# Traneptora/hydrium

Measured on AMD Instinct MI355X. Metric: Mpixel/s encode (8K RGB, default q), higher is better.
Workload: dtype f32

## Files before the change

### hydrium_amd/csrc/hip/device_api.hip

```cpp
#include <hip/hip_runtime.h>

#include <stdint.h>
#include <stdio.h>
#include <stdlib.h>
#include <string.h>

#include <atomic>
#include <condition_variable>
#include <functional>
#include <mutex>
#include <thread>
#include <vector>

#include "../../../include/hydrium_amd.h"
#include "hydk_common.h"
#include "../hyd_sample_fmt.h"

#pragma clang fp contract(off)

namespace hydk {
hipError_t launch_transform(const HydkLfJob *d_jobs, int num_slots, unsigned fmt_mask, int xmode, uint32_t *status,
                            uint2 *part_info, int plog, hipStream_t stream);
hipError_t launch_tables(const uint32_t *hist, HydkTables *tabs, const uint32_t *alpha_max, int nclusters, int first_slot,
                         int num_slots, uint32_t alpha_floor, const uint32_t *alpha_floor_dev, const uint32_t *lf_hist,
                         HydkLfStream *lf_streams, void *lf_work, const HydkLfJob *jobs_all, hipStream_t stream);
hipError_t launch_export(const HydkLfJob *d_jobs, const HydkTables *tabs, const uint32_t *group_bits, const HydkLfStream *lf_streams,
                         const uint8_t *payload, const uint64_t *hf_total, const uint8_t *lf_packed,
                         const unsigned long long *lf_total, const uint32_t *status, int num_slots, int lf_coded, uint8_t *dst,
                         uint64_t capacity, int view, hipStream_t stream);
hipError_t launch_rans(const HydkLfJob *d_jobs, const uint32_t *sym_count, const HydkTables *tabs, uint32_t *bitbuf,
                       uint32_t bit_pitch_words, uint32_t *group_bits, int num_slots, const uint32_t *status,
                       hipStream_t stream);
hipError_t launch_rans_deferred(const HydkLfJob *d_jobs, const uint32_t *sym_count, const HydkTables *tabs, uint16_t *aux,
                                uint16_t *flags, uint32_t aux_pitch, uint32_t *final_state, uint32_t *group_bits,
                                int num_slots, const uint32_t *status, hipStream_t stream);
hipError_t launch_rans_lanes(const HydkLfJob *d_jobs, const uint32_t *sym_count, const HydkTables *tabs, uint16_t *aux,
                             uint16_t *flags, uint32_t aux_pitch, uint32_t *final_state, uint32_t *group_bits,
                             int nclusters, int num_slots, const uint32_t *status, const uint32_t *lf_hist,
                             HydkLfStream *lf_streams, void *lf_work, hipStream_t stream);
hipError_t launch_lf_front(const HydkLfJob *d_jobs, unsigned long long *recs, uint32_t *hist, void *work, int num_slots,
                           hipStream_t stream);
hipError_t launch_lf_back(const HydkLfJob *d_jobs, const unsigned long long *recs, HydkLfStream *streams, uint32_t *bits,
                          void *work, int num_slots, hipStream_t stream);
hipError_t launch_rans_emit(const HydkLfJob *d_jobs, const uint32_t *sym_count, const uint16_t *aux, const uint16_t *flags,
                            uint32_t aux_pitch, const uint32_t *final_state, const uint32_t *group_bits, uint64_t *offsets,
                            uint8_t *payload, int num_slots, uint32_t *status, uint64_t *total, uint64_t payload_cap,
                            hipStream_t stream);
hipError_t launch_frame_begin(const HydkLfJob *host_jobs, HydkLfJob *d_jobs, int count, uint32_t *accum, size_t accum_words,
                              hipStream_t stream);
hipError_t launch_publish(const uint64_t *total, uint64_t *h_total, const unsigned long long *lf_total,
                          unsigned long long *h_lf_total, const uint32_t *status, uint32_t *h_status, hipStream_t stream);
hipError_t transform_footprint(int fmt, int storage, int xmode, int *lds_bytes, int *registers);
hipError_t launch_scan(const uint32_t *group_bits, int count, uint64_t *offsets, uint64_t *total, uint8_t *payload,
                       uint64_t payload_cap, int clear_shared_words, uint32_t *status, hipStream_t stream);
hipError_t launch_pack(const uint32_t *bitbuf, uint32_t bit_pitch_words, const uint32_t *group_bits, const uint64_t *offsets,
                       uint8_t *payload, int count, const uint32_t *status, hipStream_t stream);
size_t lf_work_bytes();
hipError_t launch_batch_extents(const void *blob, int frames, void *extents, hipStream_t stream);
hipError_t launch_lf_coder(const HydkLfJob *d_jobs, unsigned long long *recs, uint32_t *hist, HydkLfStream *streams,
                           uint32_t *bits, void *work, int num_slots, hipStream_t stream);
hipError_t launch_lf_gather(HydkLfStream *streams, const uint32_t *bits, uint32_t *packed, unsigned long long *total,
                            int num_slots, hipStream_t stream);
hipError_t launch_lf_huffman_only(const uint32_t *hist, HydkLfStream *stream_out, uint32_t *codes, hipStream_t stream);
hipError_t launch_lut_selftest(const uint16_t *in_lut16, const float *bias_lut, int linear_light, int xmode,
                               uint32_t *mismatches, hipStream_t stream);
}

#define ST_OK 0
#define ST_NOMEM (-13)
#define ST_API_ERROR (-14)
#define ST_INTERNAL_ERROR (-15)

static_assert(sizeof(HydAmdBlobHeader) == 64 && sizeof(HydAmdBlobSlot) == 16 + 36 + 12 + 256 + 4608 + sizeof(HydkLfStream) &&
                  sizeof(HydAmdBlobSlot) % 16 == 0,
              "blob records are laid out by k_export_frame word by word");
static_assert(HYDAMD_MAX_CLUSTERS == HYDK_MAX_CLUSTERS && HYDAMD_ALPHABET == HYDK_ALPHABET &&
                  HYDAMD_GROUPS_PER_LFG == HYDK_GROUPS_PER_LFG && HYDAMD_LF_CODES == HYDK_LF_CODES,
              "public and kernel-side table shapes must agree");

namespace {

constexpr int kStaging = 2;
constexpr int kSplitSlots = 2;
int split_slots() {
    static const int n = [] {
        const char *e = getenv("HYDAMD_K1_SPLIT_SLOTS");
        const int v = e ? atoi(e) : kSplitSlots;
        return v < 0 ? 0 : v > 256 ? 256 : v;
    }();
    return n;
}
constexpr size_t kDbgPlane = (size_t)2048 * 2048;

char g_global_error[256] = "";

struct TimedLaunch {
    int cls;
    hipEvent_t start, stop;
};

}

struct HydAmdContext {
    int device = 0;
    int max_slots = 0;
    int linear_light = 0;
    int use_luts = 2;
    int best_register_mode = 2;
    int curve_gathers = 0;
    uint64_t published_pixels = 0;
    uint64_t seen_bytes = 0, seen_pixels = 0;
    int register_luts_ok = 0;
    int rans_lanes = 0;
    uint32_t tok_cap = HYDK_DEFAULT_TOKEN_CAP;
    bool caps_forced = false;
    unsigned grown_ahead = 0;
    uint32_t rec_bytes = 4;
    uint32_t bit_pitch_words = 0;
    int want_transform = 0, want_entropy = 0;
    bool slot_lanes[HYDAMD_MAX_LF_GROUPS] = {};
    bool slot_lane_chain[HYDAMD_MAX_LF_GROUPS] = {};
    unsigned overflow_reruns = 0;
    uint32_t alpha_floor = 0;
    const uint32_t *alpha_floor_dev = nullptr;
    unsigned num_presets = 1;
    int scheme = 0;
    int nclusters = 9;
    hipStream_t own_stream = nullptr;
    hipStream_t stream = nullptr;
    char error[256] = "";

    char *tokens = nullptr;
    uint32_t *bitbuf = nullptr;
    uint16_t *rans_aux = nullptr;
    uint16_t *rans_flags = nullptr;
    uint32_t *rans_final = nullptr;
    uint32_t *rbits_total = nullptr;
    HydkTables *tables = nullptr;
    int32_t *dc = nullptr;
    uint32_t *hist = nullptr;
    uint32_t *sym_count = nullptr;
    uint2 *part_info = nullptr;
    uint32_t *group_bits = nullptr;
    uint64_t *offsets = nullptr;
    uint64_t *total = nullptr;
    uint32_t *status = nullptr;
    uint32_t *alpha_max = nullptr;
    uint32_t *bad_slots = nullptr;
    bool bad_per_slot = false;
    HydkLfJob *d_jobs = nullptr;
    HydkLfJob *h_jobs = nullptr;
    HydkLfJob *h_jobs_ring[4] = {nullptr, nullptr, nullptr, nullptr};
    hipEvent_t jobs_uploaded[4] = {nullptr, nullptr, nullptr, nullptr};
    unsigned frame_counter = 0;
    int jobs_idx = 0;
    uint16_t *in_lut8 = nullptr, *in_lut16 = nullptr;
    float *bias_lut = nullptr;
    uint8_t *payload = nullptr;
    size_t payload_cap = 0;

    int lf_on_device = 1;
    unsigned long long *lf_recs = nullptr;
    uint32_t *lf_hist = nullptr;
    uint32_t *lf_codes = nullptr;
    char *lf_work = nullptr;
    HydkLfStream *lf_streams = nullptr;
    uint32_t *lf_bits = nullptr;
    uint32_t *lf_packed = nullptr;
    unsigned long long *lf_total = nullptr;
    unsigned long long *h_lf_total_pinned = nullptr;
    uint64_t h_lf_total = 0;
    hipStream_t lf_stream = nullptr;
    hipEvent_t lf_fork = nullptr, lf_join = nullptr;
    bool lf_pending = false;
    bool lf_need_gather = false;
    bool lf_results_valid = false;
    hipEvent_t lf_ready = nullptr;
    int lf_slots = 0;
    int transformed = 0, coded = 0, lf_coded = 0;
    int host_staged = 0;
    float *dbg_xyb = nullptr, *dbg_dct = nullptr;
    int32_t *dbg_quant = nullptr;

    void *pinned[kStaging] = {nullptr, nullptr};
    char *d_arena = nullptr;
    size_t arena_tile = 0;
    size_t staging_cap = 0;
    hipEvent_t staged[kStaging] = {nullptr, nullptr};
    int staging_next = 0;
    hipStream_t copy_stream = nullptr;
    bool copy_stream_shared = false;
    hipEvent_t frame_fence = nullptr;
    bool copy_needs_fence = false;

    uint64_t h_total = 0;
    uint32_t h_status = 0;
    int slots_finished = 0;
    int slots_per_frame = 0;
    uint8_t slot_frame_first[HYDAMD_MAX_LF_GROUPS] = {};
    uint8_t slot_frame_groups[HYDAMD_MAX_LF_GROUPS] = {};
    bool results_valid = false;
    uint32_t *accum = nullptr;
    size_t accum_words = 0;
    bool accum_stale = true;
    bool lf_total_unpublished = false;
    bool status_published = false;
    uint64_t *h_total_pinned = nullptr;
    uint32_t *h_status_pinned = nullptr;

    hipEvent_t peer_event = nullptr;
    uint32_t *peer_floor = nullptr;
    unsigned long long *verify_sums = nullptr;

    void *own_blob = nullptr;
    size_t own_blob_cap = 0;
    void *stage_blob = nullptr;
    size_t stage_blob_cap = 0;
    uint8_t *stage_host = nullptr;
    size_t stage_host_cap = 0;
    int stage_slots = 0;
    HydAmdAssembler *assembler = nullptr;
    void *batch_extents = nullptr;
    size_t batch_extents_cap = 0;

    bool profiling = false;
    std::vector<TimedLaunch> timed;
    double prof_ms[HYDAMD_K_COUNT] = {0, 0, 0, 0, 0};
    uint64_t prof_n[HYDAMD_K_COUNT] = {0, 0, 0, 0, 0};
};

namespace {

int fail(HydAmdContext *ctx, int code, const char *what, hipError_t e = hipSuccess) {
    char *dst = ctx ? ctx->error : g_global_error;
    if (e != hipSuccess)
        snprintf(dst, 256, "%s: %s", what, hipGetErrorString(e));
    else
        snprintf(dst, 256, "%s", what);
    return code;
}

#define HIP_TRY(ctx, call)                                                          \
    do {                                                                            \
        hipError_t e__ = (call);                                                    \
        if (e__ != hipSuccess)                                                      \
            return fail(ctx, e__ == hipErrorOutOfMemory ? ST_NOMEM : ST_INTERNAL_ERROR, #call, e__); \
    } while (0)

float host_linearize(float x) {
    if (x <= 0.0404482362771082f)
        return 0.07739938080495357f * x;
    return 0.003094300919832f + x * (-0.009982599f + x * (0.72007737769f + 0.2852804880f * x));
}

float host_bias(float v) {
    const float x = v + 0.0037930732552754493f;
    union {
        float f;
// ... 776 lines not shown

int hydamd_set_xyb_mode(HydAmdContext *ctx, int mode) {
    if (!ctx)
        return ST_API_ERROR;
    if (recorded_but_not_transformed(ctx))
        return fail(ctx, ST_API_ERROR, "the XYB mode cannot change between recording an LF group and its transform stage");
    if (mode < ctx->best_register_mode || mode > 2)
        return fail(ctx, ST_API_ERROR, "XYB mode not available (it must have passed the bit-exactness self-test)");
    ctx->use_luts = mode;
    return ST_OK;
}

int hydamd_forget_content(HydAmdContext *ctx) {
    if (!ctx)
        return ST_API_ERROR;
    ctx->seen_bytes = ctx->seen_pixels = 0;
    return ST_OK;
}

int hydamd_set_curve_gathers(HydAmdContext *ctx, int mode) {
    if (!ctx)
        return ST_API_ERROR;
    if (mode < 0 || mode > 2)
        return fail(ctx, ST_API_ERROR, "curve gathers: 0 by content, 1 always, 2 never");
    ctx->curve_gathers = mode;
    return ST_OK;
}

int hydamd_set_rans_waves(HydAmdContext *ctx, int waves) {
    if (!ctx)
        return ST_API_ERROR;
    if (waves >= 1 && waves <= 3) {
        ctx->rans_lanes = retired_rans_form(waves);
        return ST_OK;
    }
    if (waves < 4 || waves > 6)
        return fail(ctx, ST_API_ERROR, "entropy-stage form must be 4 (wave per group) or 5 (lane per group; 6 is accepted as a synonym)");
    ctx->rans_lanes = waves - 4;
    return ST_OK;
}

int hydamd_begin_frame(HydAmdContext *ctx, unsigned num_presets) {
    if (!ctx)
        return ST_API_ERROR;
    if (num_presets < 1 || num_presets > HYDAMD_MAX_LF_GROUPS || num_presets == 128)
        return fail(ctx, ST_API_ERROR, "unsupported number of LF groups per frame (1..255 except 128)");
    HIP_TRY(ctx, hipSetDevice(ctx->device));
    ctx->num_presets = num_presets;
    if (num_presets * 9 <= 256) {
        ctx->scheme = 0;
        ctx->nclusters = 9;
    } else if (num_presets * 3 <= 256) {
        ctx->scheme = 1;
        ctx->nclusters = 3;
    } else if (num_presets * 2 <= 256) {
        ctx->scheme = 2;
        ctx->nclusters = 2;
    } else {
        ctx->scheme = 3;
        ctx->nclusters = 1;
    }
    {
        const uint32_t seen = g_outgrown.load(std::memory_order_relaxed);
        const bool tok = (seen & HYDK_STATUS_TOKENS) && ctx->tok_cap < HYDK_TOKENS_PER_GROUP;
        const bool pay = (seen & HYDK_STATUS_PAYLOAD) && ctx->payload_cap < payload_bound(ctx);
        if ((tok || pay) && !ctx->caps_forced && hipStreamQuery(ctx->stream) == hipSuccess &&
            (!ctx->lf_stream || hipStreamQuery(ctx->lf_stream) == hipSuccess)) {
            if (tok)
                ctx->tok_cap = HYDK_TOKENS_PER_GROUP;
            const int st = alloc_frame_arrays(ctx, pay ? payload_bound(ctx) : ctx->payload_cap);
            if (st != ST_OK)
                return st;
            ctx->grown_ahead++;
        }
        (void)hipGetLastError();
    }
    ctx->results_valid = false;
    ctx->slots_finished = 0;
    ctx->slots_per_frame = 0;
    ctx->transformed = ctx->coded = ctx->lf_coded = 0;
    ctx->want_transform = ctx->want_entropy = 0;
    ctx->host_staged = 0;
    ctx->lf_need_gather = false;
    ctx->lf_results_valid = false;
    ctx->lf_slots = 0;
    HIP_TRY(ctx, hipEventRecord(ctx->frame_fence, ctx->stream));
    ctx->copy_needs_fence = true;
    ctx->jobs_idx = (int)(ctx->frame_counter++ & 3u);
    HIP_TRY(ctx, hipEventSynchronize(ctx->jobs_uploaded[ctx->jobs_idx]));
    ctx->h_jobs = ctx->h_jobs_ring[ctx->jobs_idx];
    memset(ctx->h_jobs, 0, (size_t)ctx->max_slots * sizeof(HydkLfJob));
    ctx->accum_stale = true;
    ctx->alpha_floor = 0;
    ctx->alpha_floor_dev = nullptr;
    return ST_OK;
}

int hydamd_encode_lf_group(HydAmdContext *ctx, int slot, const void *const src[3], ptrdiff_t row_stride,
                           ptrdiff_t pixel_stride, int sample_fmt, size_t width, size_t height, unsigned preset) {
    int st = check_slot(ctx, slot);
    if (st != ST_OK)
        return st;
    if (!src || !src[0] || !src[1] || !src[2])
        return fail(ctx, ST_API_ERROR, "null pixel pointer");
    return record_lf_group(ctx, slot, src, row_stride, pixel_stride, sample_fmt, width, height, preset);
}

int hydamd_encode_lf_group_host(HydAmdContext *ctx, int slot, const void *const src[3], ptrdiff_t row_stride,
                                ptrdiff_t pixel_stride, int sample_fmt, size_t width, size_t height, unsigned preset) {
    int st = check_slot(ctx, slot);
    if (st != ST_OK)
        return st;
    if (!src || !src[0] || !src[1] || !src[2])
        return fail(ctx, ST_API_ERROR, "null pixel pointer");
    if (width == 0 || height == 0 || width > 2048 || height > 2048)
        return fail(ctx, ST_API_ERROR, "LF group must be between 1 and 2048 pixels in each direction");
    if (!hyd_fmt_is_host(sample_fmt))
        return fail(ctx, ST_API_ERROR, "Invalid Sample Format");
    HIP_TRY(ctx, hipSetDevice(ctx->device));
    const size_t ss = hyd_fmt_bytes(sample_fmt);
    const size_t bytes = width * height * 3 * ss;
    st = ensure_staging(ctx, (size_t)2048 * 2048 * 3 * ss);
    if (st != ST_OK)
        return st;
    const int k = ctx->staging_next;
    ctx->staging_next = (k + 1) % kStaging;
    HIP_TRY(ctx, hipEventSynchronize(ctx->staged[k]));
    if (sample_fmt == HYDK_FMT_U8)
        gather_packed((uint8_t *)ctx->pinned[k], src, row_stride, pixel_stride, width, height);
    else if (sample_fmt == HYDK_FMT_U16)
        gather_packed((uint16_t *)ctx->pinned[k], src, row_stride, pixel_stride, width, height);
    else
        gather_packed((float *)ctx->pinned[k], src, row_stride, pixel_stride, width, height);
    char *base = ctx->d_arena + (size_t)slot * ctx->arena_tile;
    if (ctx->copy_needs_fence) {
        HIP_TRY(ctx, hipStreamWaitEvent(ctx->copy_stream, ctx->frame_fence, 0));
        ctx->copy_needs_fence = false;
    }
    HIP_TRY(ctx, hipMemcpyAsync(base, ctx->pinned[k], bytes, hipMemcpyHostToDevice, ctx->copy_stream));
    HIP_TRY(ctx, hipEventRecord(ctx->staged[k], ctx->copy_stream));
    HIP_TRY(ctx, hipStreamWaitEvent(ctx->stream, ctx->staged[k], 0));
    const void *dsrc[3] = {base, base + ss, base + 2 * ss};
    st = record_lf_group(ctx, slot, dsrc, (ptrdiff_t)(3 * width), 3, sample_fmt, width, height, preset);
    if (st == ST_OK && slot + 1 > ctx->host_staged)
        ctx->host_staged = slot + 1;
    return st;
}

int hydamd_encode_image(HydAmdContext *ctx, const void *const src[3], ptrdiff_t row_stride, ptrdiff_t pixel_stride,
                        int sample_fmt, size_t width, size_t height) {
    if (!ctx)
        return ST_API_ERROR;
    if (!src || !src[0] || !src[1] || !src[2])
        return fail(ctx, ST_API_ERROR, "null pixel pointer");
    if (width == 0 || height == 0)
        return fail(ctx, ST_API_ERROR, "empty image");
    const size_t lfx = (width + 2047) >> 11, lfy = (height + 2047) >> 11;
    if (lfx * lfy > (size_t)ctx->max_slots)
        return fail(ctx, ST_API_ERROR, "context has too few LF-group slots for this image");
    if (!hyd_fmt_is_device(sample_fmt))
        return fail(ctx, ST_API_ERROR, "Invalid Sample Format");
    if (!hyd_fmt_layout_ok(sample_fmt, src, pixel_stride))
        return fail(ctx, ST_API_ERROR, HYD_FMT_NV12_LAYOUT_MSG);
    int st = hydamd_begin_frame(ctx, (unsigned)(lfx * lfy));
    for (size_t ty = 0; ty < lfy && st == ST_OK; ty++)
        for (size_t tx = 0; tx < lfx && st == ST_OK; tx++) {
// ... 43 lines not shown
            ctx->slot_frame_first[first + i] = (uint8_t)first;
            ctx->slot_frame_groups[first + i] = (uint8_t)lf_groups[k];
        }
    ctx->slots_per_frame = -1;
    return ST_OK;
}

int hydamd_encode_image_batch(HydAmdContext *ctx, int frames, const void *const *src , ptrdiff_t row_stride,
                              ptrdiff_t pixel_stride, int sample_fmt, size_t width, size_t height) {
    if (!ctx)
        return ST_API_ERROR;
    if (!src || frames < 1)
        return fail(ctx, ST_API_ERROR, "null pixel pointer");
    if (width == 0 || height == 0)
        return fail(ctx, ST_API_ERROR, "empty image");
    if (!hyd_fmt_is_device(sample_fmt))
        return fail(ctx, ST_API_ERROR, "Invalid Sample Format");
    for (int f = 0; f < frames; f++)
        if (src[3 * (size_t)f + 1] && !hyd_fmt_layout_ok(sample_fmt, src + 3 * (size_t)f, pixel_stride))
            return fail(ctx, ST_API_ERROR, HYD_FMT_NV12_LAYOUT_MSG);
    const size_t lfx = (width + 2047) >> 11, lfy = (height + 2047) >> 11, n = lfx * lfy;
    int st = hydamd_begin_batch(ctx, (unsigned)n, frames);
    for (int f = 0; f < frames && st == ST_OK; f++) {
        const void *const *s3 = src + 3 * (size_t)f;
        if (!s3[0] || !s3[1] || !s3[2])
            return fail(ctx, ST_API_ERROR, "null pixel pointer");
        for (size_t ty = 0; ty < lfy && st == ST_OK; ty++)
            for (size_t tx = 0; tx < lfx && st == ST_OK; tx++) {
                const void *p[3];
                hyd_fmt_origin(sample_fmt, s3, row_stride, pixel_stride, tx * 2048, ty * 2048, p);
                const size_t w = width - tx * 2048 < 2048 ? width - tx * 2048 : 2048;
                const size_t h = height - ty * 2048 < 2048 ? height - ty * 2048 : 2048;
                st = hydamd_encode_lf_group(ctx, (int)((size_t)f * n + ty * lfx + tx), p, row_stride, pixel_stride, sample_fmt, w, h,
                                            (unsigned)(ty * lfx + tx));
            }
    }
    if (st == ST_OK)
        st = hydamd_finish_frame(ctx, (int)((size_t)frames * n));
    return st;
}

static int transform_range(HydAmdContext *ctx, int first, int count) {
    unsigned mask = 0;
    for (int i = first; i < first + count; i++) {
        if (ctx->h_jobs[i].width == 0)
            return fail(ctx, ST_API_ERROR, "an LF-group slot of this frame was never submitted");
        mask |= 1u << (ctx->h_jobs[i].storage ? HYDK_FMT_F32 + (int)ctx->h_jobs[i].storage : ctx->h_jobs[i].fmt);
    }
    ctx->status_published = false;
    HIP_TRY(ctx, hydk::launch_frame_begin(ctx->h_jobs + first, ctx->d_jobs + first, count,
                                          ctx->accum_stale ? ctx->accum : nullptr, ctx->accum_words, ctx->stream));
    ctx->accum_stale = false;
    HIP_TRY(ctx, hipEventRecord(ctx->jobs_uploaded[ctx->jobs_idx], ctx->stream));
    ScopedTimer timer(ctx, HYDAMD_K_TRANSFORM);
    int xmode = ctx->use_luts;
    if (xmode < 2) {
        bool dense = ctx->curve_gathers == 2;
        if (ctx->curve_gathers == 0 && ctx->seen_pixels)
            dense = (double)ctx->seen_bytes > 0.75 * (double)ctx->seen_pixels;
        if (dense)
            xmode += 3;
    }
    static const bool split_on = !(getenv("HYDAMD_K1_SPLIT") && atoi(getenv("HYDAMD_K1_SPLIT")) == 0);
    static const int split_log = getenv("HYDAMD_K1_SPLIT_LOG") && atoi(getenv("HYDAMD_K1_SPLIT_LOG")) == 1 ? 1 : 2;
    const int plog = split_on && count <= split_slots() && ctx->tok_cap % 64 == 0 ? split_log : 0;
    HIP_TRY(ctx, hydk::launch_transform(ctx->d_jobs + first, count, mask, xmode, ctx->status, ctx->part_info, plog, ctx->stream));
    return ST_OK;
}

#ifdef HYD_TEST_HOOKS
static int lf_drop() {
    static const int v = getenv("HYDAMD_DEBUG_LF_DROP") ? atoi(getenv("HYDAMD_DEBUG_LF_DROP")) : 0;
    return v;
}
#else
static constexpr int lf_drop() { return 0; }
#endif
static int ensure_lf_stream(HydAmdContext *ctx) {
    if (!ctx->lf_stream)
        HIP_TRY(ctx, hipStreamCreateWithFlags(&ctx->lf_stream, hipStreamNonBlocking));
    return ST_OK;
}

static int lf_range(HydAmdContext *ctx, int first, int count, bool forked) {
    if (forked) {
        const int st = ensure_lf_stream(ctx);
        if (st != ST_OK)
            return st;
    }
    hipStream_t where = forked ? ctx->lf_stream : ctx->stream;
    ctx->status_published = false;
    if (forked) {
        HIP_TRY(ctx, hipEventRecord(ctx->lf_fork, ctx->stream));
        HIP_TRY(ctx, hipStreamWaitEvent(ctx->lf_stream, ctx->lf_fork, 0));
    }
    ScopedTimer timer(ctx, HYDAMD_K_LF, where);
    HIP_TRY(ctx, hydk::launch_lf_coder(ctx->d_jobs + first, ctx->lf_recs + (size_t)first * HYDK_LF_SYMBOLS,
                                       ctx->lf_hist + (size_t)first * HYDK_LF_CODES, ctx->lf_streams + first,
                                       ctx->lf_bits + (size_t)first * HYDK_LF_BITWORDS,
                                       ctx->lf_work + (size_t)first * hydk::lf_work_bytes(), count, where));
    ctx->lf_pending = ctx->lf_pending || forked;
    ctx->lf_need_gather = true;
    return ST_OK;
}

int hydamd_run_transform(HydAmdContext *ctx, int num_slots) {
    if (!ctx)
        return ST_API_ERROR;
    if (num_slots < 1 || num_slots > ctx->max_slots)
        return fail(ctx, ST_API_ERROR, "slot count out of range");
    HIP_TRY(ctx, hipSetDevice(ctx->device));
    ctx->results_valid = false;
    if (num_slots > ctx->want_transform)
        ctx->want_transform = num_slots;
    if (num_slots > ctx->transformed) {
        const int st = transform_range(ctx, ctx->transformed, num_slots - ctx->transformed);
        if (st != ST_OK)
            return st;
        ctx->transformed = num_slots;
    }
    if (ctx->lf_on_device == 1 && num_slots > ctx->lf_coded) {
        const int st = lf_range(ctx, ctx->lf_coded, num_slots - ctx->lf_coded, true);
        if (st != ST_OK)
            return st;
        ctx->lf_coded = num_slots;
    }
    return ST_OK;
}

static int join_lf(HydAmdContext *ctx, int num_slots, bool totals_follow = false) {
    if (num_slots > 0 && ctx->lf_on_device == 2 && num_slots > ctx->lf_coded) {
        const int st = lf_range(ctx, ctx->lf_coded, num_slots - ctx->lf_coded, false);
        if (st != ST_OK)
            return st;
        ctx->lf_coded = num_slots;
    }
    if (num_slots > 0 && ctx->lf_need_gather) {
        hipStream_t where = ctx->lf_pending ? ctx->lf_stream : ctx->stream;
        if (!(lf_drop() & 8))
        HIP_TRY(ctx, hydk::launch_lf_gather(ctx->lf_streams, ctx->lf_bits, ctx->lf_packed, ctx->lf_total, num_slots, where));
        if (totals_follow && !ctx->lf_pending)
            ctx->lf_total_unpublished = true;
        else
            HIP_TRY(ctx, hydk::launch_publish(nullptr, nullptr, ctx->lf_total, ctx->h_lf_total_pinned, nullptr, nullptr, where));
        HIP_TRY(ctx, hipEventRecord(ctx->lf_ready, where));
        ctx->lf_slots = num_slots;
        ctx->lf_need_gather = false;
    }
    if (ctx->lf_pending) {
        HIP_TRY(ctx, hipEventRecord(ctx->lf_join, ctx->lf_stream));
        HIP_TRY(ctx, hipStreamWaitEvent(ctx->stream, ctx->lf_join, 0));
        ctx->lf_pending = false;
    }
    return ST_OK;
}

static int replay_frame(HydAmdContext *ctx) {
    const int recorded = ctx->want_transform > ctx->transformed ? ctx->want_transform : ctx->transformed;
    for (int i = 0; i < ctx->max_slots; i++)
        if (ctx->h_jobs[i].width)
            bind_slot_buffers(ctx, i);
    ctx->accum_stale = true;
    const int entropy = ctx->want_entropy;
    ctx->transformed = ctx->coded = ctx->lf_coded = 0;
    ctx->results_valid = false;
    if (recorded > 0) {
        const int st = hydamd_run_transform(ctx, recorded);
        if (st != ST_OK)
            return st;
    }
    if (entropy > 0)
        return hydamd_run_entropy(ctx, entropy);
    return ST_OK;
}

static int resolve_overflow(HydAmdContext *ctx, uint32_t status, bool *again) {
    *again = false;
    if (!(status & HYDK_STATUS_OVERFLOW))
        return ST_OK;
    if (status & HYDK_STATUS_LAYOUT)
        return fail(ctx, ST_INTERNAL_ERROR, "float LF group in a context laid out for integer token records");
    if (ctx->lf_stream)
        HIP_TRY(ctx, hipStreamSynchronize(ctx->lf_stream));
    size_t payload_cap = ctx->payload_cap;
    if (status & HYDK_STATUS_TOKENS) {
// ... 565 lines not shown
                         : "vcc");
            acc = fl;
        } else {
            x = x * 1664525u + 1013904223u + row;
        }
        if (LDS) {
            const uint32_t sadr = lds0 + (__umulhi(x, lds_bytes > 2u ? lds_bytes - 2u : 1u) & ~1u);
            asm volatile("ds_read_u16 %0, %1\n\ts_waitcnt lgkmcnt(0)" : "=v"(slot) : "v"(sadr) : "memory");
            x ^= slot;
        }
        if (!VALU)
            __builtin_amdgcn_s_sleep(1);
#pragma unroll
        for (int i = 0; i < 96; i++)
            asm volatile("" : "+v"(hold[i]));
    }
    uint32_t r = x ^ acc;
#pragma unroll
    for (int i = 0; i < 96; i++)
        r ^= hold[i];
    if (r == 0xFFFFFFFFu && sink)
        *sink = r;
}
}
static int debug_skip() {
    static const int v = getenv("HYDAMD_DEBUG_SKIP") ? atoi(getenv("HYDAMD_DEBUG_SKIP")) : 0;
    return v;
}
static int env_int(const char *name, int dflt) {
    const char *v = getenv(name);
    return v && *v ? atoi(v) : dflt;
}
static void launch_chain_standins(HydAmdContext *ctx, int count) {
    static const int wgs = env_int("HYDAMD_DEBUG_SLEEP_WGS", 1);
    static const int lds = env_int("HYDAMD_DEBUG_SLEEP_LDS", 0);
    static const unsigned long long ticks = 100ull * (unsigned long long)env_int("HYDAMD_DEBUG_SLEEP_US", 2500);
    static const int regs = env_int("HYDAMD_DEBUG_SLEEP_VGPRS", 0);
    static const int steps = env_int("HYDAMD_DEBUG_STANDIN_STEPS", 30000);
    static const char *kind = getenv("HYDAMD_DEBUG_STANDIN") ? getenv("HYDAMD_DEBUG_STANDIN") : "sleep";
    const dim3 grid(wgs > 0 ? wgs * count : 1);
#define HYDK_STANDIN(MODE, THREADS)                                                                                         \
    do {                                                                                                                    \
        if (lds > 65536)                                                                                                    \
            (void)hipFuncSetAttribute((const void *)k_chain_standin, hipFuncAttributeMaxDynamicSharedMemorySize, lds);      \
        hipLaunchKernelGGL(k_chain_standin, grid, dim3(THREADS), (size_t)lds, ctx->stream, MODE, (uint32_t)steps,           \
                           (uint32_t)lds, (uint32_t *)nullptr);                                                             \
    } while (0)
    if (!strcmp(kind, "valu"))
        HYDK_STANDIN(1, 64);
    else if (!strcmp(kind, "lds"))
        HYDK_STANDIN(2, 64);
    else if (!strcmp(kind, "both"))
        HYDK_STANDIN(3, 64);
    else if (!strcmp(kind, "valu4"))
        HYDK_STANDIN(5, 256);
    else if (regs >= 160) {
        if (lds > 65536)
            (void)hipFuncSetAttribute((const void *)k_sleep_probe_regs160, hipFuncAttributeMaxDynamicSharedMemorySize, lds);
        hipLaunchKernelGGL(k_sleep_probe_regs160, grid, dim3(64), (size_t)lds, ctx->stream, ticks, (uint32_t *)nullptr);
    } else if (regs >= 124) {
        if (lds > 65536)
            (void)hipFuncSetAttribute((const void *)k_sleep_probe_regs124, hipFuncAttributeMaxDynamicSharedMemorySize, lds);
        hipLaunchKernelGGL(k_sleep_probe_regs124, grid, dim3(64), (size_t)lds, ctx->stream, ticks, (uint32_t *)nullptr);
    } else if (regs >= 100) {
        if (lds > 65536)
            (void)hipFuncSetAttribute((const void *)k_sleep_probe_regs104, hipFuncAttributeMaxDynamicSharedMemorySize, lds);
        hipLaunchKernelGGL(k_sleep_probe_regs104, grid, dim3(64), (size_t)lds, ctx->stream, ticks, (uint32_t *)nullptr);
    } else if (regs >= 40) {
        if (lds > 65536)
            (void)hipFuncSetAttribute((const void *)k_sleep_probe_regs40, hipFuncAttributeMaxDynamicSharedMemorySize, lds);
        hipLaunchKernelGGL(k_sleep_probe_regs40, grid, dim3(64), (size_t)lds, ctx->stream, ticks, (uint32_t *)nullptr);
    } else {
        if (lds > 65536)
            (void)hipFuncSetAttribute((const void *)k_sleep_probe, hipFuncAttributeMaxDynamicSharedMemorySize, lds);
        hipLaunchKernelGGL(k_sleep_probe, grid, dim3(64), (size_t)lds, ctx->stream, ticks);
    }
#undef HYDK_STANDIN
}
#else
static constexpr int debug_skip() { return 0; }
static void launch_chain_standins(HydAmdContext *, int) {}
#endif

static int entropy_range(HydAmdContext *ctx, int first, int count, bool with_lf_codes) {
    const size_t G = HYDK_GROUPS_PER_LFG, g0 = (size_t)first * G;
    {
        ScopedTimer timer(ctx, HYDAMD_K_TABLES);
        if (!(debug_skip() & 1)) {
        static const bool ride_with_tables = getenv("HYDAMD_LF_CODES_RIDE") && !strcmp(getenv("HYDAMD_LF_CODES_RIDE"), "tables");
        const bool here = with_lf_codes && ride_with_tables;
        HIP_TRY(ctx, hydk::launch_tables(ctx->hist, ctx->tables, ctx->alpha_max, ctx->nclusters, first, count,
                                         ctx->alpha_floor, ctx->alpha_floor_dev,
                                         here ? ctx->lf_hist + (size_t)first * HYDK_LF_CODES : nullptr, ctx->lf_streams + first,
                                         ctx->lf_work + (size_t)first * hydk::lf_work_bytes(), ctx->d_jobs, ctx->stream));
        if (here)
            with_lf_codes = false;
        }
    }
    {
        ScopedTimer timer(ctx, HYDAMD_K_RANS);
        const HydkLfJob *jobs = ctx->d_jobs + first;
        bool any_float = false;
        for (int i = first; i < first + count; i++)
            any_float = any_float || ctx->h_jobs[i].fmt == HYDK_FMT_F32;
        const bool lanes = ctx->rans_lanes && !any_float;
        bool emits = lanes;
        if (with_lf_codes && !lanes)
            return fail(ctx, ST_INTERNAL_ERROR, "LF code construction can only ride with the lane-form entropy stage");
        (void)lanes;
        if (debug_skip() & 16) {
            launch_chain_standins(ctx, count);
        } else if (debug_skip() & 2) {
        } else if (lanes) {
            HIP_TRY(ctx, hydk::launch_rans_lanes(jobs, ctx->sym_count + g0, ctx->tables + first,
                                                 ctx->rans_aux + g0 * ctx->tok_cap, ctx->rans_flags + g0 * (ctx->tok_cap / 16),
                                                 ctx->tok_cap, ctx->rans_final + g0, ctx->group_bits + g0,
                                                 ctx->nclusters, count, ctx->status,
                                                 with_lf_codes ? ctx->lf_hist + (size_t)first * HYDK_LF_CODES : nullptr,
                                                 ctx->lf_streams + first, ctx->lf_work + (size_t)first * hydk::lf_work_bytes(),
                                                 ctx->stream));
        } else if (!any_float && wave_form_defers()) {
            HIP_TRY(ctx, hydk::launch_rans_deferred(jobs, ctx->sym_count + g0, ctx->tables + first, ctx->rans_aux + g0 * ctx->tok_cap,
                                                    ctx->rans_flags + g0 * (ctx->tok_cap / 16), ctx->tok_cap, ctx->rans_final + g0,
                                                    ctx->group_bits + g0, count, ctx->status, ctx->stream));
            emits = true;
        } else {
            const int st = ensure_bitbuf(ctx);
            if (st != ST_OK)
                return st;
            HIP_TRY(ctx, hydk::launch_rans(jobs, ctx->sym_count + g0, ctx->tables + first,
                                           ctx->bitbuf + g0 * ctx->bit_pitch_words, ctx->bit_pitch_words,
                                           ctx->group_bits + g0, count, ctx->status, ctx->stream));
        }
        for (int i = first; i < first + count; i++) {
            ctx->slot_lanes[i] = emits;
            ctx->slot_lane_chain[i] = lanes;
        }
    }
    return ST_OK;
}

int hydamd_run_entropy(HydAmdContext *ctx, int num_slots) {
    if (!ctx)
        return ST_API_ERROR;
    if (num_slots < 1 || num_slots > ctx->max_slots)
        return fail(ctx, ST_API_ERROR, "slot count out of range");
    if (num_slots > ctx->transformed)
        return fail(ctx, ST_API_ERROR, "the entropy stage needs the transform stage of the same slots first");
    HIP_TRY(ctx, hipSetDevice(ctx->device));
    const int count = num_slots * HYDK_GROUPS_PER_LFG;
    ctx->results_valid = false;
    ctx->want_entropy = num_slots;
    int lf_first = -1, lf_count = 0;
    if (num_slots > ctx->coded && ctx->lf_on_device == 2 && ctx->rans_lanes && ctx->lf_coded == ctx->coded && !ctx->lf_pending &&
        !(debug_skip() & 8)) {
        bool any_float = false;
        for (int i = ctx->coded; i < num_slots; i++)
            any_float = any_float || ctx->h_jobs[i].fmt == HYDK_FMT_F32;
        if (!any_float) {
            lf_first = ctx->coded;
            lf_count = num_slots - ctx->coded;
            ScopedTimer timer(ctx, HYDAMD_K_LF);
            if (!(lf_drop() & 1))
            HIP_TRY(ctx, hydk::launch_lf_front(ctx->d_jobs + lf_first, ctx->lf_recs + (size_t)lf_first * HYDK_LF_SYMBOLS,
                                               ctx->lf_hist + (size_t)lf_first * HYDK_LF_CODES,
                                               ctx->lf_work + (size_t)lf_first * hydk::lf_work_bytes(), lf_count, ctx->stream));
        }
    }
    if (num_slots > ctx->coded) {
        const int st = entropy_range(ctx, ctx->coded, num_slots - ctx->coded, lf_count > 0 && !(lf_drop() & 2));
        if (st != ST_OK)
            return st;
        ctx->coded = num_slots;
    }
    if (!(debug_skip() & 4)) {
        ScopedTimer timer(ctx, HYDAMD_K_PACK);
        bool all_emit = true;
        for (int i = 0; i < num_slots; i++)
            all_emit = all_emit && ctx->slot_lane_chain[i];
        if (all_emit)
            HIP_TRY(ctx, hydk::launch_rans_emit(ctx->d_jobs, ctx->sym_count, ctx->rans_aux, ctx->rans_flags, ctx->tok_cap,
                                                ctx->rans_final, ctx->group_bits, ctx->offsets, ctx->payload, num_slots,
                                                ctx->status, ctx->total, ctx->payload_cap, ctx->stream));
        else
            HIP_TRY(ctx, hydk::launch_scan(ctx->group_bits, count, ctx->offsets, ctx->total, ctx->payload, ctx->payload_cap, 1,
                                           ctx->status, ctx->stream));
        for (int first = all_emit ? num_slots : 0; first < num_slots;) {
            int last = first;
            while (last + 1 < num_slots && ctx->slot_lanes[last + 1] == ctx->slot_lanes[first])
                last++;
            const int n = last - first + 1;
            const size_t g0 = (size_t)first * HYDK_GROUPS_PER_LFG;
            if (ctx->slot_lanes[first])
                HIP_TRY(ctx, hydk::launch_rans_emit(ctx->d_jobs + first, ctx->sym_count + g0, ctx->rans_aux + g0 * ctx->tok_cap,
                                                    ctx->rans_flags + g0 * (ctx->tok_cap / 16), ctx->tok_cap,
                                                    ctx->rans_final + g0, ctx->group_bits + g0, ctx->offsets + g0, ctx->payload,
                                                    n, ctx->status, nullptr, 0, ctx->stream));
            else
                HIP_TRY(ctx, hydk::launch_pack(ctx->bitbuf + g0 * ctx->bit_pitch_words, ctx->bit_pitch_words,
                                               ctx->group_bits + g0, ctx->offsets + g0, ctx->payload,
                                               n * HYDK_GROUPS_PER_LFG, ctx->status, ctx->stream));
            first = last + 1;
        }
    }
    if (lf_count > 0) {
        ScopedTimer timer(ctx, HYDAMD_K_LF);
        if (!(lf_drop() & 4))
        HIP_TRY(ctx, hydk::launch_lf_back(ctx->d_jobs + lf_first, ctx->lf_recs + (size_t)lf_first * HYDK_LF_SYMBOLS,
                                          ctx->lf_streams + lf_first, ctx->lf_bits + (size_t)lf_first * HYDK_LF_BITWORDS,
                                          ctx->lf_work + (size_t)lf_first * hydk::lf_work_bytes(), lf_count, ctx->stream));
        ctx->lf_coded = num_slots;
        ctx->lf_need_gather = true;
    }
    {
        const int st = join_lf(ctx, num_slots, true);
        if (st != ST_OK)
            return st;
    }
    {
        uint64_t px = 0;
        for (int i = 0; i < num_slots; i++)
            px += (uint64_t)ctx->h_jobs[i].width * (uint64_t)ctx->h_jobs[i].height;
        ctx->published_pixels = px;
    }
    HIP_TRY(ctx, hydk::launch_publish(ctx->total, ctx->h_total_pinned, ctx->lf_total_unpublished ? ctx->lf_total : nullptr,
                                      ctx->h_lf_total_pinned, ctx->status, ctx->h_status_pinned, ctx->stream));
#ifdef HYD_TEST_HOOKS
    {
        static const int extra = env_int("HYDAMD_DEBUG_EXTRA_LAUNCHES", 0);
        for (int i = 0; i < extra; i++)
            HIP_TRY(ctx, hydk::launch_publish(nullptr, nullptr, nullptr, nullptr, nullptr, nullptr, ctx->stream));
    }
#endif
    if (ctx->lf_total_unpublished)
        HIP_TRY(ctx, hipEventRecord(ctx->lf_ready, ctx->stream));
    ctx->lf_total_unpublished = false;
    ctx->status_published = true;
    ctx->slots_finished = num_slots;
    return ST_OK;
}

int hydamd_submit_lf_group(HydAmdContext *ctx, int slot) {
    int st = check_slot(ctx, slot);
    if (st != ST_OK)
        return st;
    if (slot != ctx->transformed)
        return fail(ctx, ST_API_ERROR, "LF groups are submitted early in slot order, one at a time");
    HIP_TRY(ctx, hipSetDevice(ctx->device));
    ctx->results_valid = false;
    st = transform_range(ctx, slot, 1);
    if (st == ST_OK)
        ctx->transformed = slot + 1;
    return st;
}

int hydamd_run_lf_coder(HydAmdContext *ctx, int num_slots, int last) {
    if (!ctx)
        return ST_API_ERROR;
    if (!ctx->lf_on_device)
        return fail(ctx, ST_API_ERROR, "the LF coder is off");
    if (num_slots < 1 || num_slots > ctx->max_slots)
        return fail(ctx, ST_API_ERROR, "slot count out of range");
    HIP_TRY(ctx, hipSetDevice(ctx->device));
    ctx->results_valid = false;
    if (num_slots > ctx->transformed) {
        const int st = transform_range(ctx, ctx->transformed, num_slots - ctx->transformed);
        if (st != ST_OK)
            return st;
        ctx->transformed = num_slots;
    }
    if (ctx->lf_pending) {
        HIP_TRY(ctx, hipEventRecord(ctx->lf_join, ctx->lf_stream));
        HIP_TRY(ctx, hipStreamWaitEvent(ctx->stream, ctx->lf_join, 0));
        ctx->lf_pending = false;
    }
    if (num_slots > ctx->lf_coded) {
        const int st = lf_range(ctx, ctx->lf_coded, num_slots - ctx->lf_coded, false);
        if (st != ST_OK)
            return st;
        ctx->lf_coded = num_slots;
    }
    return last ? join_lf(ctx, num_slots) : ST_OK;
}

int hydamd_sync_lf(HydAmdContext *ctx) {
    if (!ctx)
        return ST_API_ERROR;
    if (!ctx->lf_on_device || ctx->lf_need_gather || ctx->lf_slots == 0)
        return fail(ctx, ST_API_ERROR, "no finished LF coder run to wait for");
    HIP_TRY(ctx, hipSetDevice(ctx->device));
    HIP_TRY(ctx, hipEventSynchronize(ctx->lf_ready));
    ctx->h_lf_total = *ctx->h_lf_total_pinned;
    ctx->lf_results_valid = true;
    return ST_OK;
}
// ... 176 lines not shown
        for (int c = 0; c < 3; c++)
            rgb[3 * i + c] = (uint8_t)out[c];
    }
    return ST_OK;
}

namespace {
__global__ __launch_bounds__(256) void k_yuv_to_rgb_probe(int matrix, const uint8_t *yuv, uint8_t *rgb, size_t n) {
    const size_t i = (size_t)blockIdx.x * 256u + threadIdx.x;
    if (i >= n)
        return;
    uint32_t out[3];
    hydk_yuv_to_rgb(hydk_yuv_matrix(matrix), yuv[3 * i], yuv[3 * i + 1], yuv[3 * i + 2], out);
    for (int c = 0; c < 3; c++)
        rgb[3 * i + c] = (uint8_t)out[c];
}
}

__attribute__((visibility("default"))) int hydt_yuv_to_rgb_device(int device, int matrix, const uint8_t *yuv, uint8_t *rgb, size_t n) {
    if (matrix < 0 || matrix >= HYDK_YUV_MATRICES || !yuv || !rgb || n == 0 || n >= ((size_t)1 << 31) ||
        hipSetDevice(device) != hipSuccess)
        return ST_API_ERROR;
    uint8_t *d_in = nullptr, *d_out = nullptr;
    hipError_t e = hipMalloc((void **)&d_in, 3 * n);
    if (e == hipSuccess)
        e = hipMalloc((void **)&d_out, 3 * n);
    if (e == hipSuccess)
        e = hipMemcpy(d_in, yuv, 3 * n, hipMemcpyHostToDevice);
    if (e == hipSuccess) {
        hipLaunchKernelGGL(k_yuv_to_rgb_probe, dim3((unsigned)((n + 255) / 256)), dim3(256), 0, nullptr, matrix, d_in, d_out, n);
        e = hipGetLastError();
    }
    if (e == hipSuccess)
        e = hipMemcpy(rgb, d_out, 3 * n, hipMemcpyDeviceToHost);
    (void)hipFree(d_in);
    (void)hipFree(d_out);
    return e == hipSuccess ? ST_OK : ST_API_ERROR;
}
#endif

int hydamd_set_lf_coder(HydAmdContext *ctx, int on_device) {
    if (!ctx)
        return ST_API_ERROR;
    ctx->lf_on_device = on_device == 2 ? 2 : on_device != 0;
    return ST_OK;
}

int hydamd_lf_coder(HydAmdContext *ctx) { return ctx ? ctx->lf_on_device : 0; }

int hydamd_read_lf_stream(HydAmdContext *ctx, int slot, uint8_t lengths[HYDAMD_LF_CODES], uint32_t *alphabet,
                          uint32_t *run_pairs, uint32_t *bit_count) {
    int st = check_slot(ctx, slot);
    if (st != ST_OK)
        return st;
    if (!ctx->lf_on_device || !ctx->lf_results_valid)
        return fail(ctx, ST_API_ERROR, "no device-coded LF stream: the LF coder is off or the frame was not synchronised");
    HydkLfStream h;
    HIP_TRY(ctx, hipMemcpy(&h, ctx->lf_streams + slot, sizeof(h), hipMemcpyDeviceToHost));
    if (h.error)
        return fail(ctx, ST_INTERNAL_ERROR, "LF code construction failed on the device");
    memcpy(lengths, h.lengths, HYDK_LF_CODES);
    if (alphabet)
        *alphabet = h.alphabet;
    if (run_pairs)
        *run_pairs = h.run_pairs;
    if (bit_count)
        *bit_count = h.bit_count;
    return ST_OK;
}

int hydamd_read_lf_bits(HydAmdContext *ctx, int slot, uint8_t *dst, size_t capacity) {
    int st = check_slot(ctx, slot);
    if (st != ST_OK)
        return st;
    if (!ctx->lf_on_device || !ctx->lf_results_valid)
        return fail(ctx, ST_API_ERROR, "no device-coded LF stream: the LF coder is off or the frame was not synchronised");
    if (capacity > (size_t)HYDK_LF_BITWORDS * sizeof(uint32_t))
        return fail(ctx, ST_API_ERROR, "LF bit request too large");
    if (!capacity)
        return ST_OK;
    HydkLfStream h;
    HIP_TRY(ctx, hipMemcpy(&h, ctx->lf_streams + slot, sizeof(h), hipMemcpyDeviceToHost));
    const size_t have = ((size_t)h.bit_count + 7u) / 8u, n = capacity < have ? capacity : have;
    if (n)
        HIP_TRY(ctx, hipMemcpy(dst, ctx->lf_bits + (size_t)slot * HYDK_LF_BITWORDS, n, hipMemcpyDeviceToHost));
    memset(dst + n, 0, capacity - n);
    return ST_OK;
}

size_t hydamd_lf_payload_size(HydAmdContext *ctx) {
    return ctx && ctx->lf_results_valid && ctx->lf_on_device ? (size_t)ctx->h_lf_total : 0;
}

const uint8_t *hydamd_lf_payload_device(HydAmdContext *ctx) { return ctx ? (const uint8_t *)ctx->lf_packed : nullptr; }

int hydamd_read_lf_payload(HydAmdContext *ctx, uint8_t *dst, size_t capacity) {
    if (!ctx || !ctx->lf_on_device || !ctx->lf_results_valid)
        return fail(ctx, ST_API_ERROR, "no device-coded LF stream: the LF coder is off or the frame was not synchronised");
    if (capacity < ctx->h_lf_total)
        return fail(ctx, ST_API_ERROR, "LF payload buffer too small");
    if (ctx->h_lf_total)
        HIP_TRY(ctx, hipMemcpy(dst, ctx->lf_packed, ctx->h_lf_total, hipMemcpyDeviceToHost));
    return ST_OK;
}

int hydamd_read_lf_streams(HydAmdContext *ctx, int first_slot, int count, HydAmdLfInfo *dst) {
    if (!ctx || !ctx->lf_on_device || !ctx->lf_results_valid)
        return fail(ctx, ST_API_ERROR, "no device-coded LF stream: the LF coder is off or the frame was not synchronised");
    if (first_slot < 0 || count < 1 || first_slot + count > ctx->lf_slots)
        return fail(ctx, ST_API_ERROR, "LF-group slot range out of bounds");
    static_assert(sizeof(HydAmdLfInfo) == sizeof(HydkLfStream), "public and kernel-side LF stream records must agree");
    HIP_TRY(ctx, hipMemcpy(dst, ctx->lf_streams + first_slot, (size_t)count * sizeof(HydkLfStream), hipMemcpyDeviceToHost));
    for (int i = 0; i < count; i++)
        if (dst[i].error)
            return fail(ctx, ST_INTERNAL_ERROR, "LF code construction failed on the device");
    return ST_OK;
}

int hydamd_debug_transform_footprint(HydAmdContext *ctx, int sample_fmt, int *lds_bytes, int *registers) {
    if (!ctx || !lds_bytes || !registers || !hyd_fmt_is_device(sample_fmt))
        return ST_API_ERROR;
    HIP_TRY(ctx, hipSetDevice(ctx->device));
    HIP_TRY(ctx, hydk::transform_footprint(fmt_class(sample_fmt), (int)fmt_storage(sample_fmt), ctx->use_luts, lds_bytes, registers));
    return ST_OK;
}

namespace {
__global__ __launch_bounds__(64) void k_clock_probe(unsigned long long *out) {
    const unsigned long long r0 = __builtin_amdgcn_s_memrealtime();
    const unsigned long long c0 = __builtin_amdgcn_s_memtime();
    unsigned long long r1 = r0;
    while (r1 - r0 < 2000ull)
        r1 = __builtin_amdgcn_s_memrealtime();
    const unsigned long long c1 = __builtin_amdgcn_s_memtime();
    if (threadIdx.x == 0) {
        out[0] = c1 - c0;
        out[1] = r1 - r0;
    }
}
}

int hydamd_debug_shader_clock_mhz(HydAmdContext *ctx, double *mhz) {
    if (!ctx || !mhz)
        return ST_API_ERROR;
    HIP_TRY(ctx, hipSetDevice(ctx->device));
    static std::mutex lock;
    static hipStream_t sides[HYDAMD_MAX_PEERS * 2];
    static unsigned long long *pinned[HYDAMD_MAX_PEERS * 2];
    if (ctx->device < 0 || ctx->device >= HYDAMD_MAX_PEERS * 2)
        return fail(ctx, ST_API_ERROR, "device index out of range");
    std::lock_guard<std::mutex> hold(lock);
    hipStream_t &side = sides[ctx->device];
    unsigned long long *&h = pinned[ctx->device];
    if (!side)
        HIP_TRY(ctx, hipStreamCreateWithFlags(&side, hipStreamNonBlocking));
    if (!h)
        HIP_TRY(ctx, hipHostMalloc((void **)&h, 2 * sizeof(unsigned long long), hipHostMallocDefault));
    hipLaunchKernelGGL(k_clock_probe, dim3(1), dim3(64), 0, side, h);
    HIP_TRY(ctx, hipGetLastError());
    HIP_TRY(ctx, hipStreamSynchronize(side));
    *mhz = h[1] ? 100.0 * (double)h[0] / (double)h[1] : 0.0;
    return ST_OK;
}

int hydamd_debug_lf_code(HydAmdContext *ctx, const uint32_t hist[HYDAMD_LF_CODES], uint8_t lengths[HYDAMD_LF_CODES],
                         uint32_t codes[HYDAMD_LF_CODES], uint32_t *alphabet, uint32_t *error) {
    if (!ctx)
        return ST_API_ERROR;
// ... 92 lines not shown
```

### hydrium_amd/csrc/hip/kernels.hip

```cpp
#include <hip/hip_runtime.h>
#include <stdint.h>

#include "hydk_common.h"
#include "hydk_edges.h"
#include <atomic>
#include <type_traits>

#pragma clang fp contract(off)

namespace {

constexpr int kThreads = 256;
#ifndef HYDK_K1_WAVES
#define HYDK_K1_WAVES 4
#endif
#ifndef HYDK_K1_GATHER
#define HYDK_K1_GATHER 0x10
#endif
#ifndef HYDK_K1_WAVELOCAL
#define HYDK_K1_WAVELOCAL 1
#endif
#ifndef HYDK_K1_SKIP
#define HYDK_K1_SKIP 0
#endif
// ... 1017 lines not shown
                    uint32_t token, rbits, residue;
                    if (FMT != HYDK_FMT_F32) {
                        const uint32_t fb = __float_as_uint((float)value) >> 22;
                        const bool big = value >= 16u;
                        token = big ? fb - 246u : value;
                        rbits = big ? (fb >> 1) - 128u : 0u;
                        residue = __builtin_amdgcn_ubfe(value, 0u, rbits);
                    } else if (value < 16) {
                        token = value;
                        rbits = 0;
                        residue = 0;
                    } else {
                        const int nb = 30 - __clz((int)value);
                        rbits = (uint32_t)nb;
                        residue = value & ((1u << nb) - 1u);
                        token = 16u + (((uint32_t)(nb - 3) << 1) | ((value >> nb) & 1u));
                    }
#if HYDK_K1_TRIM
                    const uint32_t bin = umad24(cluster, (uint32_t)kHistW, FMT == HYDK_FMT_F32 ? min(token, (uint32_t)kHistW - 1u) : token);
#else
                    const uint32_t bin = cluster * kHistW + (FMT == HYDK_FMT_F32 ? min(token, (uint32_t)kHistW - 1u) : token);
#endif
                    store_record<FMT>(tok, goff + p, token, cluster, bin, rbits, residue);
                    rb_sum += rbits;
                    atomicAdd(&s_hist[bin], 1u);
                    const uint32_t here = coef != 0 ? 1u : 0u;
                    remaining -= here;
                    prev = is_count ? (uint32_t)(nz_total <= 4u) : here;
                    if (++j == n) {
                        seg_at++;
                        visit = visit == 2u ? 0u : visit + 1u;
                        seg = s_seg[seg_at];
                        n = seg.z & 0xffu;
                        nz_total = remaining = seg.z >> 8;
                        j = 0;
                    }
                }
            }
        }
        goff += strip_total;
        __syncthreads();
    }

    __syncthreads();
    uint32_t top_token = 0;
    for (int i = t; i < HYDK_MAX_CLUSTERS * kHistW; i += kThreads) {
        const uint32_t v = s_hist[i];
        if (v) {
            atomicAdd(&job.hist[(i / kHistW) * HYDK_ALPHABET + i % kHistW], v);
            top_token = max(top_token, (uint32_t)(i % kHistW) + 1u);
        }
    }
#pragma unroll
    for (int d = 32; d; d >>= 1)
        top_token = max(top_token, (uint32_t)__shfl_xor((int)top_token, d));
    if (lane == 0 && top_token)
        atomicMax(job.alpha_max, top_token);
#pragma unroll
    for (int d = 32; d; d >>= 1)
        rb_sum += (uint32_t)__shfl_xor((int)rb_sum, d);
    if (lane == 0)
        atomicAdd(&s_rbits, rb_sum);
    __syncthreads();
    if (t == 0) {
        const uint32_t count = overflowed || HYDK_K1_SKIP ? 0u : goff;
        if (plog) {
            part_info[blockIdx.x] = uint2{count, s_rbits};
        } else {
            job.sym_count[g] = count;
            job.rbits_total[g] = s_rbits;
        }
        if (overflowed)
            atomicOr(status, HYDK_STATUS_TOKENS);
    }
    if (FMT == HYDK_FMT_F32 && bad_sample) {
        if (job.bad_slot)
            atomicOr(job.bad_slot, 1u);
        else
            atomicOr(status, HYDK_STATUS_BAD_SAMPLE);
    }
}

#include "lf_huffman.h"

__global__ __launch_bounds__(kThreads) void k_join_parts(const HydkLfJob *__restrict__ jobs, const uint2 *part_info, int plog,
                                                         uint32_t *status) {
    const HydkLfJob job = jobs[blockIdx.x >> 6];
    const int g = blockIdx.x & 63;
    if (g >= job.gcols * job.grows)
        return;
    const uint32_t parts = 1u << plog, room = job.tok_cap >> plog, wpr = job.fmt == HYDK_FMT_F32 ? 2u : 1u;
    uint32_t *const base = (uint32_t *)((char *)job.tokens + (size_t)g * job.tok_cap * job.rec_bytes);
    bool bogus = false;
    uint2 p0 = part_info[(size_t)blockIdx.x * parts];
    if (p0.x > room) {
        p0 = uint2{0u, 0u};
        bogus = true;
    }
    uint32_t total = p0.x, rbits = p0.y;
    for (uint32_t q = 1; q < parts; q++) {
        uint2 pi = part_info[(size_t)blockIdx.x * parts + q];
        if (pi.x > room) {
            pi = uint2{0u, 0u};
            bogus = true;
        }
        const uint32_t *src = base + (size_t)q * room * wpr;
        uint32_t *dst = base + (size_t)total * wpr;
        const uint32_t words = pi.x * wpr;
        if (dst != src) {
            constexpr uint32_t kPer = 8;
            for (uint32_t at = 0; at < words; at += kPer * kThreads) {
                uint32_t v[kPer];
#pragma unroll
                for (uint32_t k = 0; k < kPer; k++) {
                    const uint32_t i = at + k * kThreads + threadIdx.x;
                    v[k] = i < words ? src[i] : 0u;
                }
                __syncthreads();
#pragma unroll
                for (uint32_t k = 0; k < kPer; k++) {
                    const uint32_t i = at + k * kThreads + threadIdx.x;
                    if (i < words)
                        dst[i] = v[k];
                }
            }
        }
        total += pi.x;
        rbits += pi.y;
    }
    if (threadIdx.x == 0) {
        job.sym_count[g] = bogus ? 0u : total;
        job.rbits_total[g] = bogus ? 0u : rbits;
        if (bogus)
            atomicOr(status, HYDK_STATUS_INCONSISTENT);
    }
}

__global__ __launch_bounds__(kThreads) void k_build_tables(const uint32_t *hist_all, HydkTables *tabs,
                                                           const uint32_t *alpha_max_all, int nclusters,
                                                           uint32_t alpha_floor, const uint32_t *alpha_floor_dev,
                                                           int first_slot, int num_slots, const uint32_t *lf_hist,
                                                           HydkLfStream *lf_streams, void *lf_work, const HydkLfJob *__restrict__ jobs_all) {
    HYDK_URGENT();
    if ((int)blockIdx.x >= num_slots) {
        __shared__ LfHuffScratch s_huff;
        const int s = (int)blockIdx.x - num_slots;
        if (threadIdx.x < 64)
            lf_code_and_offsets_wave(lf_hist + (size_t)s * HYDK_LF_CODES, ((LfWork *)lf_work)[s], lf_streams + s,
                                     jobs_all[first_slot + s], s_huff, (int)threadIdx.x);
        return;
    }
    const unsigned slot = (unsigned)first_slot + blockIdx.x;
    const uint32_t *hist = hist_all + (size_t)slot * HYDK_MAX_CLUSTERS * HYDK_ALPHABET;
    HydkTables *tab = tabs + slot;
    __shared__ uint32_t s_freq[HYDK_MAX_CLUSTERS][HYDK_ALPHABET];
    __shared__ uint32_t s_cutoff[HYDK_MAX_CLUSTERS][HYDK_ALPHABET];
    __shared__ uint32_t s_other[HYDK_MAX_CLUSTERS][HYDK_ALPHABET];
    __shared__ uint32_t s_shift[HYDK_MAX_CLUSTERS][HYDK_ALPHABET];
    __shared__ uint32_t s_base[HYDK_MAX_CLUSTERS][HYDK_ALPHABET];
    __shared__ uint8_t s_under[HYDK_MAX_CLUSTERS][HYDK_ALPHABET];
    __shared__ uint8_t s_over[HYDK_MAX_CLUSTERS][HYDK_ALPHABET];
    __shared__ uint32_t s_alpha[HYDK_MAX_CLUSTERS];
    __shared__ uint32_t s_log_alpha, s_err;

    const int t = threadIdx.x;
    for (int i = t; i < HYDK_MAX_CLUSTERS * HYDK_ALPHABET; i += kThreads) {
        (&s_freq[0][0])[i] = hist[i];
        (&s_cutoff[0][0])[i] = 0;
        (&s_other[0][0])[i] = 0;
        (&s_shift[0][0])[i] = 0;
        (&s_base[0][0])[i] = 0;
    }
    if (t == 0)
        s_err = 0;
    __syncthreads();

    if (t < HYDK_MAX_CLUSTERS) {
        uint32_t a = 0;
        if (t < nclusters)
            for (int k = 0; k < HYDK_ALPHABET; k++)
                if (s_freq[t][k])
                    a = k + 1;
        s_alpha[t] = a;
    }
    __syncthreads();
    if (t == 0) {
        uint32_t mx = alpha_floor;
        if (alpha_floor_dev)
            mx = max(mx, *alpha_floor_dev);
        const unsigned frame_first = min((unsigned)jobs_all[slot].frame_first, slot);
        for (unsigned sl = frame_first; sl <= slot; sl++)
            mx = max(mx, alpha_max_all[sl]);
        uint32_t lg = mx > 1 ? 32 - __clz((int)(mx - 1)) : 0;
        s_log_alpha = max(lg, 5u);
        tab->running_max_alphabet = mx;
    }
    __syncthreads();
    const int log_alpha = (int)s_log_alpha;
    const int log_bucket = 12 - log_alpha;
    const uint32_t bucket = 1u << log_bucket, table_size = 1u << log_alpha;

    if (t < nclusters && s_alpha[t]) {
        uint32_t *f = s_freq[t];
        const uint32_t n = s_alpha[t];
        unsigned long long total = 0;
        for (uint32_t k = 0; k < n; k++)
            total += f[k];
        unsigned long long scaled = 0;
        for (uint32_t k = 0; k < n; k++) {
            if (!f[k])
                continue;
            uint32_t v = (uint32_t)((((unsigned long long)f[k] << 12) / total) & 0xFFFFu);
            if (!v)
                v = 1;
            f[k] = v;
            scaled += v;
        }
        int j = (int)n - 1;
        while (scaled > 4096 && j >= 0) {
            const unsigned long long excess = scaled - 4096;
            if (excess < f[j]) {
                f[j] -= (uint32_t)excess;
                scaled -= excess;
                break;
            } else if (f[j] > 1) {
                scaled -= f[j] - 1;
                f[j] = 1;
            }
            j--;
        }
        f[0] += (uint32_t)(4096 - scaled);
        const bool unique = f[n - 1] == 4096;

        uint32_t *cutoff = s_cutoff[t], *other = s_other[t], *shift = s_shift[t];
        if (unique) {
            for (uint32_t i = 0; i < table_size; i++) {
                other[i] = n - 1;
                shift[i] = i * bucket;
            }
        } else {
            uint8_t *under = s_under[t], *over = s_over[t];
            uint32_t nu = 0, no = 0;
            for (uint32_t sidx = 0; sidx < n; sidx++) {
                cutoff[sidx] = f[sidx];
                if (f[sidx] < bucket)
                    under[nu++] = (uint8_t)sidx;
// ... 798 lines not shown
#define HYDK_LANE_FETCH(F, AHEAD)                                                                                \
    do {                                                                                                         \
        if (rj - (AHEAD) >= 0 && !(HYDK_CHAIN_PROBE & (4 | 16))) {                                               \
            _Pragma("unroll") for (int q = 0; q < 4; q++) F[q] = load_records4(tok, (rj - (AHEAD)) * 4 + q);     \
        }                                                                                                        \
    } while (0)

    uint32_t pw[8] = {0, 0, 0, 0, 0, 0, 0, 0}, pfl = 0;
    int prj = -1;
    int it = 0;
#if HYDK_LANE_PIPE == 1
    uint4 nb[4] = {};
#define HYDK_LANE_TURN(FIRST, C, F)                                                                              \
    if (it < rounds) {                                                                                           \
        __builtin_amdgcn_s_waitcnt(0x0F70);                                        \
        HYDK_LANE_ROUND(FIRST, C, HYDK_LANE_FETCH(F, 1); HYDK_LANE_STORE_PREV());                                \
        it++;                                                                                                    \
    }
    HYDK_LANE_TURN(true, nx, nb)
    while (it < rounds) {
        HYDK_LANE_TURN(false, nb, nx)
        HYDK_LANE_TURN(false, nx, nb)
    }
#else
    uint4 ny[4], nb[4] = {}, nc[4] = {};
#pragma unroll
    for (int q = 0; q < 4; q++)
        ny[q] = rj >= 1 && !(HYDK_CHAIN_PROBE & 4) ? load_records4(tok, (rj - 1) * 4 + q) : uint4{0, 0, 0, 0};
#define HYDK_LANE_TURN(FIRST, C0, C1, F0, F1)                                                                    \
    if (it < rounds) {                                                                                           \
                                                      \
        __builtin_amdgcn_s_waitcnt(0x0F70);                                                        \
        HYDK_LANE_ROUND(FIRST, C0, HYDK_LANE_FETCH(F0, 2); HYDK_LANE_FETCH(F1, 3); HYDK_LANE_STORE_PREV());      \
        it++;                                                                                                    \
        if (it < rounds) {                                                                                       \
            HYDK_LANE_ROUND(false, C1, HYDK_LANE_STORE_PREV());                                                  \
            it++;                                                                                                \
        }                                                                                                        \
    }
    HYDK_LANE_TURN(true, nx, ny, nb, nc)
    while (it < rounds) {
        HYDK_LANE_TURN(false, nb, nc, nx, ny)
        HYDK_LANE_TURN(false, nx, ny, nb, nc)
    }
#endif
#undef HYDK_LANE_TURN
#undef HYDK_LANE_FETCH
#undef HYDK_LANE_ROUND
    HYDK_LANE_STORE_PREV();
#undef HYDK_LANE_STORE_PREV
#endif
#undef HYDK_LANE_STEP_TAIL
#undef HYDK_LANE_STEP_BODY
#undef HYDK_LANE_STEP_HEAD
#undef HYDK_LANE_STEP_COLD
#undef HYDK_LANE_COLD_SLOT
#undef HYDK_LANE_ROW
    if (lane < ngroups) {
        final_state_all[G] = state;
        group_bits_all[G] = (uint32_t)jobs[slot].preset_bits + (n > 0 ? 32u : 0u) + 16u * refills + HYDK_GLOBAL(const uint32_t, jobs[slot].rbits_total)[lane];
    } else {
        group_bits_all[G] = 0;
    }
#if HYDK_CHAIN_PROBE & 32
    if (lane == 0)
        group_bits_all[G] = probe_t0;
    if (lane == 1)
        group_bits_all[G] = (uint32_t)__builtin_amdgcn_s_memrealtime();
#endif
}

#ifndef HYDK_EMIT_SHARE_DEFAULT
#define HYDK_EMIT_SHARE_DEFAULT 1
#endif
constexpr int kEmitPer = 8;
constexpr int kEmitBatch = 64 * kEmitPer;
constexpr int kEmitWin = kEmitBatch + 4;

template <bool SELF>
__global__ __launch_bounds__(kThreads) void k_rans_emit(const HydkLfJob *__restrict__ jobs, const uint32_t *sym_count_all,
                                                        const uint16_t *aux_all, const uint16_t *flags_all, uint32_t aux_pitch,
                                                        const uint32_t *final_state_all, const uint32_t *group_bits_all,
                                                        uint64_t *offsets_all, uint8_t *payload, uint32_t *status, int vblocks,
                                                        uint64_t *total, uint64_t payload_cap) {
    __shared__ uint32_t s_win[4][kEmitWin];
    HYDK_URGENT();
    const int t = threadIdx.x, lane = t & 63, wave = t >> 6;
    auto wave_sum = [](uint64_t v) {
        const uint32_t lo = __builtin_amdgcn_readlane(scan64_inclusive((uint32_t)v & 0xFFFFFFu), 63);
        const uint32_t hi = __builtin_amdgcn_readlane(scan64_inclusive((uint32_t)(v >> 24)), 63);
        return ((uint64_t)hi << 24) + lo;
    };
    uint64_t all = 0;
    bool fits = true;
    if (SELF) {
        uint64_t mine_all = 0;
        for (int i = lane; i < vblocks * 4; i += 64)
            mine_all += (group_bits_all[i] + 7u) >> 3;
        all = wave_sum(mine_all);
        fits = all <= payload_cap && !(*status & HYDK_STATUS_OVERFLOW);
    }
    auto one_block = [&](const int vb) {
    const int slot = vb >> 4;
    const int g = ((vb & 15) << 2) + wave;
    const int ngroups = jobs[slot].gcols * jobs[slot].grows;
    const size_t G = (size_t)slot * HYDK_GROUPS_PER_LFG + g;
    uint64_t sec_lo = 0;
    if (SELF) {
        uint64_t mine_before = 0;
        for (size_t i = lane; i < G; i += 64)
            mine_before += (group_bits_all[i] + 7u) >> 3;
        sec_lo = wave_sum(mine_before);
        if (lane == 0) {
            offsets_all[G] = sec_lo;
            if (G == 0) {
                *total = fits ? all : 0;
                if (all > payload_cap)
                    atomicOr(status, HYDK_STATUS_PAYLOAD);
                if (fits)
                    for (uint64_t b = all; b & 3u; b++)
                        payload[b] = 0;
            }
        }
        if (g >= ngroups || !fits)
            return;
    } else if (g >= ngroups || (*status & HYDK_STATUS_OVERFLOW))
        return;
    const void *tok = (const char *)jobs[slot].tokens + (size_t)g * jobs[slot].tok_cap * jobs[slot].rec_bytes;
    const uint4 *aux = (const uint4 *)(aux_all + G * aux_pitch);
    const uint16_t *flags = flags_all + G * (aux_pitch / 16);
    uint32_t *W = (uint32_t *)payload;
    uint32_t *win = s_win[wave];
    const int n = __builtin_amdgcn_readfirstlane((int)sym_count_all[G]);
    const uint32_t bits = group_bits_all[G];
    const unsigned long long lo_bit = (SELF ? sec_lo : offsets_all[G]) * 8ull, hi_bit = lo_bit + (unsigned long long)((bits + 7u) & ~7u);
    const uint32_t shared_lo = (lo_bit & 31ull) ? (uint32_t)(lo_bit >> 5) : 0xFFFFFFFFu;
    const uint32_t shared_hi = (hi_bit & 31ull) ? (uint32_t)((hi_bit - 1ull) >> 5) : 0xFFFFFFFFu;
    const uint32_t wbase = (uint32_t)(lo_bit >> 5);
    uint32_t cur = (uint32_t)(lo_bit & 31ull) + bits;
    uint32_t carry = 0;

    bool bad = false;
    auto put = [&](uint32_t word, uint32_t v) {
        const uint32_t d = wbase + word;
        if (SELF && (d == shared_lo || d == shared_hi))
            hydk_store_edge_word(payload, d, v, lo_bit >> 3, hi_bit >> 3);
        else if (d == shared_lo || d == shared_hi)
            atomicOr(&W[d], v);
        else
            W[d] = v;
    };
    auto emit = [&](const uint32_t (&val)[kEmitPer], const uint32_t (&nb)[kEmitPer], auto &&before_stores) {
        uint32_t mine = 0;
#pragma unroll
        for (int j = 0; j < kEmitPer; j++)
            mine += nb[j];
        const uint32_t inc = scan64_inclusive(mine);
        const uint32_t total = __builtin_amdgcn_readlane(inc, 63);
        if (!total) {
            before_stores();
            return;
        }
        if (total > cur) {
            if (lane == 0)
                atomicOr(status, HYDK_STATUS_INCONSISTENT);
            bad = true;
            return;
        }
// ... 15 lines not shown
                if ((uint32_t)lo)
                    atomicOr(&win[w], (uint32_t)lo);
                if ((uint32_t)(lo >> 32))
                    atomicOr(&win[w + 1], (uint32_t)(lo >> 32));
            }
            pos += nb[j];
        }
        __builtin_amdgcn_wave_barrier();
        before_stores();
        const bool low_partial = (newcur & 31u) != 0;
        for (uint32_t i = lane + (low_partial ? 1u : 0u); i < nwords; i += 64)
            put(wlo + i, win[i]);
        carry = low_partial ? win[0] : 0u;
        __builtin_amdgcn_wave_barrier();
        cur = newcur;
    };

    uint4 rec_n[2] = {{0, 0, 0, 0}, {0, 0, 0, 0}};
    uint4 a_n = {0, 0, 0, 0};
    uint32_t fl_n = 0;
    auto fetch = [&](int batch) {
        const int p0 = batch * kEmitBatch + kEmitPer * lane;
        if (batch >= 0 && p0 < n) {
            rec_n[0] = load_records4(tok, p0 >> 2);
            rec_n[1] = load_records4(tok, (p0 >> 2) + 1);
            a_n = aux[p0 >> 3];
            fl_n = flags[p0 >> 4];
        }
    };
    const int batches = (n + kEmitBatch - 1) / kEmitBatch;
    uint32_t rc[kEmitPer] = {0, 0, 0, 0, 0, 0, 0, 0}, ac[4] = {0, 0, 0, 0}, flc = 0;
    auto take = [&] {
        const uint32_t r[kEmitPer] = {rec_n[0].x, rec_n[0].y, rec_n[0].z, rec_n[0].w, rec_n[1].x, rec_n[1].y, rec_n[1].z, rec_n[1].w};
        const uint32_t a[4] = {a_n.x, a_n.y, a_n.z, a_n.w};
#pragma unroll
        for (int j = 0; j < kEmitPer; j++) {
            rc[j] = r[j];
            asm volatile("" : "+v"(rc[j]));
        }
#pragma unroll
        for (int j = 0; j < 4; j++) {
            ac[j] = a[j];
            asm volatile("" : "+v"(ac[j]));
        }
        flc = fl_n;
        asm volatile("" : "+v"(flc));
    };
    fetch(batches - 1);
    take();
    for (int b = batches - 1; b >= 0; b--) {
        const int p0 = b * kEmitBatch + kEmitPer * lane;
        const uint32_t recs[kEmitPer] = {rc[0], rc[1], rc[2], rc[3], rc[4], rc[5], rc[6], rc[7]};
        const uint32_t aw[kEmitPer] = {ac[0] & 0xFFFFu, ac[0] >> 16, ac[1] & 0xFFFFu, ac[1] >> 16,
                                       ac[2] & 0xFFFFu, ac[2] >> 16, ac[3] & 0xFFFFu, ac[3] >> 16};
        const uint32_t flq = flc >> (p0 & 15);
        fetch(b - 1);
        uint32_t val[kEmitPer], nb[kEmitPer];
#pragma unroll
        for (int j = 0; j < kEmitPer; j++) {
            const bool valid = p0 + j < n;
            const bool refill = valid && ((flq >> j) & 1u);
            const uint32_t rbits = HYDK_REC32_RBITS(recs[j]), residue = recs[j] >> 16;
            val[j] = refill ? (residue << 16) | aw[j] : residue;
            nb[j] = valid ? rbits + (refill ? 16u : 0u) : 0u;
        }
        emit(val, nb, take);
        if (bad) return;
    }
    {
        uint32_t val[kEmitPer] = {0, 0, 0, 0, 0, 0, 0, 0}, nb[kEmitPer] = {0, 0, 0, 0, 0, 0, 0, 0};
        if (lane == 0) {
            val[0] = jobs[slot].preset;
            nb[0] = (uint32_t)jobs[slot].preset_bits;
            if (n > 0) {
                val[1] = final_state_all[G];
                nb[1] = 32;
            }
        }
        emit(val, nb, [] {});
    }
    if (lane == 0 && (cur & 31u))
        put(cur >> 5, carry);
    };
    for (int vb = blockIdx.x; vb < vblocks; vb += gridDim.x)
        one_block(vb);
}

__global__ __launch_bounds__(kThreads) void k_frame_begin(const uint32_t *__restrict__ host_jobs, uint32_t *__restrict__ d_jobs,
                                                          uint32_t job_words, uint4 *__restrict__ accum, uint32_t quads) {
    HYDK_URGENT();
    if (blockIdx.x == 0) {
        for (uint32_t i = threadIdx.x; i < job_words; i += kThreads)
            d_jobs[i] = host_jobs[i];
        return;
    }
    for (uint32_t i = (blockIdx.x - 1) * kThreads + threadIdx.x; i < quads; i += (gridDim.x - 1) * kThreads)
        accum[i] = make_uint4(0u, 0u, 0u, 0u);
}

__global__ __launch_bounds__(64) void k_publish(const uint64_t *total, uint64_t *h_total, const unsigned long long *lf_total,
                                                unsigned long long *h_lf_total, const uint32_t *status, uint32_t *h_status) {
    HYDK_URGENT();
    if (threadIdx.x == 0 && total)
        *h_total = *total;
    if (threadIdx.x == 1 && lf_total)
        *h_lf_total = *lf_total;
    if (threadIdx.x == 2 && status)
        *h_status = *status;
}

__global__ __launch_bounds__(kThreads) void k_scan_sections(const uint32_t *group_bits, int count, uint64_t *offsets,
                                                            uint64_t *total, uint8_t *payload, uint64_t payload_cap,
                                                            int clear_shared_words, uint32_t *status) {
    __shared__ uint64_t s_wave[4];
    HYDK_URGENT();
    const int t = threadIdx.x, lane = t & 63, wave = t >> 6;
    const int per = (count + kThreads - 1) / kThreads;
    const int lo = min(count, t * per), hi = min(count, lo + per);
    uint64_t sum = 0;
    for (int i = lo; i < hi; i++)
        sum += (group_bits[i] + 7u) >> 3;
    uint64_t inc = sum;
#pragma unroll
    for (int d = 1; d < 64; d <<= 1) {
        const uint64_t v = __shfl_up(inc, d);
        if (lane >= d)
            inc += v;
    }
    if (lane == 63)
        s_wave[wave] = inc;
    __syncthreads();
    uint64_t before = 0, all = 0;
    for (int w = 0; w < 4; w++) {
        before += w < wave ? s_wave[w] : 0;
        all += s_wave[w];
    }
    const bool fits = all <= payload_cap && !(*status & HYDK_STATUS_OVERFLOW);
    uint64_t run = before + inc - sum;
    for (int i = lo; i < hi; i++) {
        const uint64_t nbytes = (group_bits[i] + 7u) >> 3;
        offsets[i] = run;
        if (clear_shared_words && fits && nbytes) {
            if (run & 3u)
                ((uint32_t *)payload)[run >> 2] = 0;
            if ((run + nbytes) & 3u)
                ((uint32_t *)payload)[(run + nbytes - 1) >> 2] = 0;
        }
        run += nbytes;
    }
    if (t == kThreads - 1) {
        *total = fits ? all : 0;
        if (all > payload_cap)
            atomicOr(status, HYDK_STATUS_PAYLOAD);
    }
}

__global__ __launch_bounds__(kThreads) void k_pack_sections(const uint32_t *bitbuf, uint32_t bit_pitch_words,
                                                            const uint32_t *group_bits, const uint64_t *offsets,
                                                            uint8_t *payload, const uint32_t *status) {
    const int G = blockIdx.x;
    const uint32_t bits = group_bits[G];
    if (!bits || (*status & HYDK_STATUS_OVERFLOW))
        return;
    const uint32_t nbytes = (bits + 7u) >> 3;
    const uint32_t *W = bitbuf + (size_t)G * bit_pitch_words;
    const uint32_t start = bit_pitch_words * 32u - bits;
    const uint32_t sw = start >> 5, sh = start & 31u;
// ... 114 lines not shown
    do {                                       \
        if (xmode == kXybFastRcp)              \
            HYDK_LAUNCH_K1(FMT, kXybFastRcp);  \
        else if (xmode == kXybIeeeDiv)         \
            HYDK_LAUNCH_K1(FMT, kXybIeeeDiv);  \
        else if (xmode == kXybFastRcpRegs)     \
            HYDK_LAUNCH_K1(FMT, kXybFastRcpRegs); \
        else if (xmode == kXybIeeeDivRegs)     \
            HYDK_LAUNCH_K1(FMT, kXybIeeeDivRegs); \
        else                                   \
            HYDK_LAUNCH_K1(FMT, kXybGather);   \
    } while (0)
    if (fmt_mask & (1u << HYDK_FMT_U8))
        HYDK_LAUNCH_K1_MODES(HYDK_FMT_U8);
    if (fmt_mask & (1u << HYDK_FMT_U16))
        HYDK_LAUNCH_K1_MODES(HYDK_FMT_U16);
#define HYDK_LAUNCH_K1_FLOAT(STORE)                       \
    if (fmt_mask & (1u << (HYDK_FMT_F32 + (STORE))))      \
    hipLaunchKernelGGL((k_transform_tokenize<HYDK_FMT_F32, kXybIeeeDiv, STORE>), grid, block, 0, stream, d_jobs, status, part_info, plog)
    HYDK_LAUNCH_K1_FLOAT(HYDK_STORE_F32);
    HYDK_LAUNCH_K1_FLOAT(HYDK_STORE_F16);
    HYDK_LAUNCH_K1_FLOAT(HYDK_STORE_BF16);
#undef HYDK_LAUNCH_K1_FLOAT
    if (fmt_mask & (1u << (HYDK_FMT_F32 + HYDK_STORE_NV12))) {
#define HYDK_LAUNCH_K1_NV12(XM) \
    hipLaunchKernelGGL((k_transform_tokenize<HYDK_FMT_U8, XM, HYDK_STORE_NV12>), grid, block, 0, stream, d_jobs, status, part_info, plog)
        if (xyb_arith(xmode) == kXybFastRcp)
            HYDK_LAUNCH_K1_NV12(kXybFastRcp);
        else if (xyb_arith(xmode) == kXybIeeeDiv)
            HYDK_LAUNCH_K1_NV12(kXybIeeeDiv);
        else
            HYDK_LAUNCH_K1_NV12(kXybGather);
#undef HYDK_LAUNCH_K1_NV12
    }
#undef HYDK_LAUNCH_K1_MODES
#undef HYDK_LAUNCH_K1
    if (plog)
        hipLaunchKernelGGL(k_join_parts, dim3(num_slots * HYDK_GROUPS_PER_LFG), block, 0, stream, d_jobs, part_info, plog, status);
    return hipGetLastError();
}

hipError_t transform_footprint(int fmt, int storage, int xmode, int *lds_bytes, int *registers) {
    const void *fn = nullptr;
#define HYDK_K1_PTR(FMT, XM) fn = (const void *)k_transform_tokenize<FMT, XM>
    if (fmt == HYDK_FMT_F32 && storage == HYDK_STORE_F16)
        fn = (const void *)k_transform_tokenize<HYDK_FMT_F32, kXybIeeeDiv, HYDK_STORE_F16>;
    else if (fmt == HYDK_FMT_F32 && storage == HYDK_STORE_BF16)
        fn = (const void *)k_transform_tokenize<HYDK_FMT_F32, kXybIeeeDiv, HYDK_STORE_BF16>;
    else if (fmt == HYDK_FMT_F32)
        HYDK_K1_PTR(HYDK_FMT_F32, kXybIeeeDiv);
    else if (fmt == HYDK_FMT_U8 && storage == HYDK_STORE_NV12) {
        if (xmode == kXybFastRcp)
            fn = (const void *)k_transform_tokenize<HYDK_FMT_U8, kXybFastRcp, HYDK_STORE_NV12>;
        else if (xmode == kXybIeeeDiv)
            fn = (const void *)k_transform_tokenize<HYDK_FMT_U8, kXybIeeeDiv, HYDK_STORE_NV12>;
        else
            fn = (const void *)k_transform_tokenize<HYDK_FMT_U8, kXybGather, HYDK_STORE_NV12>;
    } else if (fmt == HYDK_FMT_U8) {
        if (xmode == kXybFastRcp)
            HYDK_K1_PTR(HYDK_FMT_U8, kXybFastRcp);
        else if (xmode == kXybIeeeDiv)
            HYDK_K1_PTR(HYDK_FMT_U8, kXybIeeeDiv);
        else
            HYDK_K1_PTR(HYDK_FMT_U8, kXybGather);
    } else {
        if (xmode == kXybFastRcp)
            HYDK_K1_PTR(HYDK_FMT_U16, kXybFastRcp);
        else if (xmode == kXybIeeeDiv)
            HYDK_K1_PTR(HYDK_FMT_U16, kXybIeeeDiv);
        else
            HYDK_K1_PTR(HYDK_FMT_U16, kXybGather);
    }
#undef HYDK_K1_PTR
    hipFuncAttributes attr;
    const hipError_t e = hipFuncGetAttributes(&attr, fn);
    if (e == hipSuccess) {
        *lds_bytes = (int)attr.sharedSizeBytes;
        *registers = attr.numRegs;
    }
    return e;
}

hipError_t launch_tables(const uint32_t *hist, HydkTables *tabs, const uint32_t *alpha_max, int nclusters, int first_slot,
                         int num_slots, uint32_t alpha_floor, const uint32_t *alpha_floor_dev, const uint32_t *lf_hist,
                         HydkLfStream *lf_streams, void *lf_work, const HydkLfJob *jobs_all, hipStream_t stream) {
    hipLaunchKernelGGL(k_build_tables, dim3(lf_hist ? 2 * num_slots : num_slots), dim3(kThreads), 0, stream, hist, tabs, alpha_max,
                       nclusters, alpha_floor, alpha_floor_dev, first_slot, num_slots, lf_hist, lf_streams, lf_work, jobs_all);
    return hipGetLastError();
}

hipError_t launch_rans(const HydkLfJob *d_jobs, const uint32_t *sym_count, const HydkTables *tabs, uint32_t *bitbuf,
                       uint32_t bit_pitch_words, uint32_t *group_bits, int num_slots, const uint32_t *status,
                       hipStream_t stream) {
    hipLaunchKernelGGL((k_rans_encode<4, false>), dim3(num_slots * 16), dim3(256), 0, stream, d_jobs, sym_count, tabs, bitbuf,
                       bit_pitch_words, group_bits, status, (uint16_t *)nullptr, (uint16_t *)nullptr, 0u,
                       (uint32_t *)nullptr);
    return hipGetLastError();
}

hipError_t launch_rans_deferred(const HydkLfJob *d_jobs, const uint32_t *sym_count, const HydkTables *tabs, uint16_t *aux,
                                uint16_t *flags, uint32_t aux_pitch, uint32_t *final_state, uint32_t *group_bits,
                                int num_slots, const uint32_t *status, hipStream_t stream) {
    hipLaunchKernelGGL((k_rans_encode<4, true>), dim3(num_slots * 16), dim3(256), 0, stream, d_jobs, sym_count, tabs,
                       (uint32_t *)nullptr, 0u, group_bits, status, aux, flags, aux_pitch, final_state);
    return hipGetLastError();
}

hipError_t launch_rans_lanes(const HydkLfJob *d_jobs, const uint32_t *sym_count, const HydkTables *tabs, uint16_t *aux,
                             uint16_t *flags, uint32_t aux_pitch, uint32_t *final_state, uint32_t *group_bits,
                             int nclusters, int num_slots, const uint32_t *status, const uint32_t *lf_hist,
                             HydkLfStream *lf_streams, void *lf_work, hipStream_t stream) {
    const dim3 grid(lf_hist ? 2 * num_slots : num_slots);
#if HYDK_CHAIN_DYN_LDS
#define HYDK_LAUNCH_LANES(NC)                                                                                                  \
    do {                                                                                                                       \
         \
        static std::atomic<uint32_t> opted{0};                                                                                 \
        int dev = 0;                                                                                                           \
        if (lanes_lds_bytes(NC) > 65536 && hipGetDevice(&dev) == hipSuccess && !((opted.load() >> (dev & 31)) & 1u)) {         \
            const hipError_t e = hipFuncSetAttribute((const void *)k_rans_lanes<NC>, hipFuncAttributeMaxDynamicSharedMemorySize, lanes_lds_bytes(NC)); \
            if (e != hipSuccess)                                                                                               \
                return e;                                                                                                      \
            opted.fetch_or(1u << (dev & 31));                                                                                  \
        }                                                                                                                      \
        hipLaunchKernelGGL(k_rans_lanes<NC>, grid, dim3(64), (size_t)lanes_lds_bytes(NC), stream, d_jobs, sym_count, tabs, aux, flags, aux_pitch, \
                           final_state, group_bits, status, num_slots, lf_hist, lf_streams, lf_work);                          \
    } while (0)
#else
#define HYDK_LAUNCH_LANES(NC)                                                                                                  \
    hipLaunchKernelGGL(k_rans_lanes<NC>, grid, dim3(64), 0, stream, d_jobs, sym_count, tabs, aux, flags, aux_pitch, final_state, \
                       group_bits, status, num_slots, lf_hist, lf_streams, lf_work)
#endif
    if (nclusters == 9)
        HYDK_LAUNCH_LANES(HYDK_LANE_NC9_PROBE);
    else if (nclusters == 3)
        HYDK_LAUNCH_LANES(3);
    else if (nclusters == 2)
        HYDK_LAUNCH_LANES(2);
    else if (nclusters == 1)
        HYDK_LAUNCH_LANES(1);
    else
        return hipErrorInvalidValue;
#undef HYDK_LAUNCH_LANES
    return hipGetLastError();
}

hipError_t launch_rans_emit(const HydkLfJob *d_jobs, const uint32_t *sym_count, const uint16_t *aux, const uint16_t *flags,
                            uint32_t aux_pitch, const uint32_t *final_state, const uint32_t *group_bits, uint64_t *offsets,
                            uint8_t *payload, int num_slots, uint32_t *status, uint64_t *total, uint64_t payload_cap,
                            hipStream_t stream) {
    static const int share = [] {
        const char *v = getenv("HYDAMD_EMIT_SHARE");
        const int n = v && *v ? atoi(v) : HYDK_EMIT_SHARE_DEFAULT;
        return n < 1 ? 1 : n > 16 ? 16 : n;
    }();
    const int vblocks = num_slots * 16;
    const dim3 grid((vblocks + share - 1) / share);
    if (total)
        hipLaunchKernelGGL(k_rans_emit<true>, grid, dim3(kThreads), 0, stream, d_jobs, sym_count, aux, flags, aux_pitch, final_state,
                           group_bits, offsets, payload, status, vblocks, total, payload_cap);
    else
        hipLaunchKernelGGL(k_rans_emit<false>, grid, dim3(kThreads), 0, stream, d_jobs, sym_count, aux, flags, aux_pitch,
                           final_state, group_bits, offsets, payload, status, vblocks, (uint64_t *)nullptr, (uint64_t)0);
    return hipGetLastError();
}

hipError_t launch_frame_begin(const HydkLfJob *host_jobs, HydkLfJob *d_jobs, int count, uint32_t *accum, size_t accum_words,
                              hipStream_t stream) {
    const uint32_t quads = accum ? (uint32_t)(accum_words / 4) : 0u;
    const uint32_t job_words = (uint32_t)((size_t)count * sizeof(HydkLfJob) / sizeof(uint32_t));
    const uint32_t blocks = 1u + (quads + kThreads - 1) / kThreads;
    hipLaunchKernelGGL(k_frame_begin, dim3(blocks < 64u ? blocks : 64u), dim3(kThreads), 0, stream, (const uint32_t *)host_jobs,
                       (uint32_t *)d_jobs, job_words, (uint4 *)accum, quads);
    return hipGetLastError();
}

hipError_t launch_publish(const uint64_t *total, uint64_t *h_total, const unsigned long long *lf_total,
                          unsigned long long *h_lf_total, const uint32_t *status, uint32_t *h_status, hipStream_t stream) {
    hipLaunchKernelGGL(k_publish, dim3(1), dim3(64), 0, stream, total, h_total, lf_total, h_lf_total, status, h_status);
    return hipGetLastError();
}

hipError_t launch_scan(const uint32_t *group_bits, int count, uint64_t *offsets, uint64_t *total, uint8_t *payload,
                       uint64_t payload_cap, int clear_shared_words, uint32_t *status, hipStream_t stream) {
    hipLaunchKernelGGL(k_scan_sections, dim3(1), dim3(kThreads), 0, stream, group_bits, count, offsets, total, payload, payload_cap,
                       clear_shared_words, status);
    return hipGetLastError();
}

hipError_t launch_pack(const uint32_t *bitbuf, uint32_t bit_pitch_words, const uint32_t *group_bits, const uint64_t *offsets,
                       uint8_t *payload, int count, const uint32_t *status, hipStream_t stream) {
    hipLaunchKernelGGL(k_pack_sections, dim3(count), dim3(kThreads), 0, stream, bitbuf, bit_pitch_words, group_bits, offsets,
                       payload, status);
    return hipGetLastError();
}

hipError_t launch_export(const HydkLfJob *d_jobs, const HydkTables *tabs, const uint32_t *group_bits, const HydkLfStream *lf_streams,
                         const uint8_t *payload, const uint64_t *hf_total, const uint8_t *lf_packed,
                         const unsigned long long *lf_total, const uint32_t *status, int num_slots, int lf_coded, uint8_t *dst,
                         uint64_t capacity, int view, hipStream_t stream) {
    hipLaunchKernelGGL(k_export_frame, dim3(num_slots + 1 + (view ? 0 : kExportCopyBlocks)), dim3(kThreads), 0, stream, d_jobs, tabs,
                       group_bits, lf_streams, payload, hf_total, lf_packed, lf_total, status, num_slots, lf_coded, dst, capacity, view);
    return hipGetLastError();
}

hipError_t launch_lut_selftest(const uint16_t *in_lut16, const float *bias_lut, int linear_light, int xmode,
                               uint32_t *mismatches, hipStream_t stream) {
    if (xmode == kXybFastRcp)
        hipLaunchKernelGGL(k_lut_selftest<kXybFastRcp>, dim3(256), dim3(256), 0, stream, in_lut16, bias_lut, linear_light,
                           mismatches);
    else
        hipLaunchKernelGGL(k_lut_selftest<kXybIeeeDiv>, dim3(256), dim3(256), 0, stream, in_lut16, bias_lut, linear_light,
                           mismatches);
    return hipGetLastError();
}

}
```

### hydrium_amd/csrc/hip/lf_coder.hip

```cpp
#include <hip/hip_runtime.h>

#include <stdint.h>

#include "hydk_common.h"
#ifndef HYDK_LF_WPB
#define HYDK_LF_WPB 1
#endif
#ifndef HYDK_LF_PROBE
#define HYDK_LF_PROBE 0
#endif

namespace {

#include "lf_huffman.h"

constexpr int kPlane = HYDK_DC_PITCH * HYDK_DC_PITCH;

#define LF_REC(v, lit, r) ((unsigned long long)(v) | ((unsigned long long)((uint32_t)(lit) | ((uint32_t)(r) << 1)) << 32))

struct LfShape {
    int vbw, blocks, n;
    uint32_t vbw_magic;
};

__device__ __forceinline__ LfShape lf_shape(const HydkLfJob &job) {
    LfShape sh;
    sh.vbw = (job.width + 7) >> 3;
    sh.blocks = sh.vbw * ((job.height + 7) >> 3);
    sh.n = lf_values_of(job);
    sh.vbw_magic = sh.vbw > 1 ? (uint32_t)(0xFFFFFFFFu / (uint32_t)sh.vbw) + 1u : 0u;
    return sh;
}

__device__ __forceinline__ int lf_row_of(const LfShape &sh, int rem) {
    return sh.vbw > 1 ? (int)__umulhi((uint32_t)rem, sh.vbw_magic) : rem;
}

__device__ __forceinline__ void lf_hybrid(uint32_t v, uint32_t &token, uint32_t &nbits, uint32_t &residue) {
    if (v < 128u) {
        token = v;
        nbits = 0;
        residue = 0;
        return;
    }
    const uint32_t nb = (31u - (uint32_t)__clz(v)) - 2u;
    residue = (v >> 1) & ((1u << nb) - 1u);
    token = 128u + (((nb - 5u) << 2) | (((v >> (nb + 1u)) & 1u) << 1) | (v & 1u));
    nbits = nb;
}

#define LF_DPP_KEEP(v, ctrl, rmask) ((uint32_t)__builtin_amdgcn_update_dpp((int)(v), (int)(v), ctrl, rmask, 0xF, false))

__device__ __forceinline__ int wave_incl_max(int v) {
    int t;
    t = (int)LF_DPP_KEEP(v, 0x111, 0xF);
    v = v > t ? v : t;
    t = (int)LF_DPP_KEEP(v, 0x112, 0xF);
    v = v > t ? v : t;
    t = (int)LF_DPP_KEEP(v, 0x114, 0xF);
    v = v > t ? v : t;
    t = (int)LF_DPP_KEEP(v, 0x118, 0xF);
    v = v > t ? v : t;
    t = (int)LF_DPP_KEEP(v, 0x142, 0xA);
    v = v > t ? v : t;
    t = (int)LF_DPP_KEEP(v, 0x143, 0xC);
    v = v > t ? v : t;
    return v;
}

struct LfTokenScratch {
    int wtot[kLfWaves];
    uint32_t lastv[kLfWaves];
    int head[kLfWaves];
    uint32_t first;
};

__device__ __forceinline__ uint32_t lf_predict(int32_t cur, int32_t w, int32_t n, int32_t nw) {
    const int32_t lo = w < n ? w : n, hi = w < n ? n : w;
    int32_t pred = (int32_t)((uint32_t)w + (uint32_t)n - (uint32_t)nw);
    pred = pred < lo ? lo : pred > hi ? hi : pred;
    const uint32_t d = (uint32_t)cur - (uint32_t)pred;
    return (d << 1) ^ (0u - (d >> 31));
}

__device__ __forceinline__ uint32_t lf_residual_at(const int32_t *dc, int c, int y, int x) {
    const int idx = c * kPlane + y * HYDK_DC_PITCH + x;
    const int iw = x ? idx - 1 : y ? idx - HYDK_DC_PITCH : idx;
    const int in = y ? idx - HYDK_DC_PITCH : iw;
    const int inw = x && y ? idx - HYDK_DC_PITCH - 1 : iw;
    const int32_t cur = dc[idx];
    int32_t w = dc[iw], n = dc[in], nw = dc[inw];
    if (!(x | y))
        w = n = nw = 0;
    return lf_predict(cur, w, n, nw);
}

__device__ __forceinline__ uint32_t lf_value_at(const int32_t *dc, const LfShape &sh, int i) {
    const int visit = (i >= sh.blocks) + (i >= 2 * sh.blocks);
    const int rem = i - visit * sh.blocks;
    const int y = lf_row_of(sh, rem), x = rem - y * sh.vbw;
    return lf_residual_at(dc, visit < 2 ? 1 - visit : 2, y, x);
}

__device__ __forceinline__ void lf_fetch(const int32_t *dc, const LfShape &sh, int i0, uint32_t (&v)[4]) {
#pragma unroll
    for (int j = 0; j < 4; j++)
        v[j] = 0;
    if (i0 >= sh.n)
        return;
    int visit = (i0 >= sh.blocks) + (i0 >= 2 * sh.blocks);
    const int rem = i0 - visit * sh.blocks;
    int y = lf_row_of(sh, rem), x = rem - y * sh.vbw;
    if (x + 3 < sh.vbw) {
        const int c = visit < 2 ? 1 - visit : 2;
        const int32_t *row = dc + c * kPlane + y * HYDK_DC_PITCH + x;
        const int32_t *up = y ? row - HYDK_DC_PITCH : row;
        const int32_t c0 = row[0], c1 = row[1], c2 = row[2], c3 = row[3];
        const int32_t u0 = up[0], u1 = up[1], u2 = up[2], u3 = up[3];
        const int32_t left = row[x ? -1 : 0], upleft = up[x ? -1 : 0];
        const int32_t w0 = x ? left : y ? u0 : 0;
        v[0] = lf_predict(c0, w0, y ? u0 : w0, y && x ? upleft : w0);
        v[1] = lf_predict(c1, c0, y ? u1 : c0, y ? u0 : c0);
        v[2] = lf_predict(c2, c1, y ? u2 : c1, y ? u1 : c1);
        v[3] = lf_predict(c3, c2, y ? u3 : c2, y ? u2 : c2);
        return;
    }
    const int vbh = sh.blocks / sh.vbw;
#pragma unroll
    for (int j = 0; j < 4; j++) {
        if (visit < 3)
            v[j] = lf_residual_at(dc, visit < 2 ? 1 - visit : 2, y, x);
        if (++x == sh.vbw) {
            x = 0;
            if (++y == vbh) {
                y = 0;
                visit++;
            }
        }
    }
}

__device__ __forceinline__ int lf_run_start(const int32_t *dc, const LfShape &sh, int from, LfTokenScratch &S) {
    const int tid = threadIdx.x, lane = tid & 63, wave = tid >> 6;
    for (int top = from; top >= 0; top -= kLfThreads) {
        const int p = top - tid;
        int head = -1;
        if (p >= 0)
            head = (p == 0 || lf_value_at(dc, sh, p) != lf_value_at(dc, sh, p - 1)) ? p : -1;
        head = wave_incl_max(head);
        if (lane == 63)
            S.head[wave] = head;
        __syncthreads();
        int best = -1;
#pragma unroll
        for (int w = 0; w < kLfWaves; w++)
            best = best > S.head[w] ? best : S.head[w];
        __syncthreads();
        if (best >= 0)
            return best;
    }
    return 0;
}

__device__ __forceinline__ uint32_t lf_tokens_window(const HydkLfJob &job, const LfShape &sh, unsigned long long *__restrict__ recs,
                                                     int tb, int *s_rs , uint32_t *s_hist, LfTokenScratch &S) {
    const int tid = threadIdx.x, lane = tid & 63, wave = tid >> 6;
    const int32_t *dc = job.dc;
    const int q0 = tid * 4;

    for (int i = tid; i < HYDK_LF_CODES; i += kLfThreads)
        s_hist[i] = 0;
    uint32_t v[4];
    lf_fetch(dc, sh, tb + q0, v);
    const uint32_t tailv = tb > 0 ? lf_value_at(dc, sh, tb - 1) : 0u;
    if (lane == 63)
        S.lastv[wave] = v[3];
    if (tid == 0)
        S.first = v[0];
    __syncthreads();
    const bool continues = tb > 0 && tb < sh.n && S.first == tailv;
    const int carry = continues ? lf_run_start(dc, sh, tb - 1, S) : 0;

    uint32_t prev = LF_DPP_KEEP(v[3], 0x138, 0xF);
    if (lane == 0)
        prev = wave ? S.lastv[wave - 1] : tailv;
    int rs[4];
    int last = -1;
#pragma unroll
    for (int j = 0; j < 4; j++) {
        const int i = tb + q0 + j;
        last = (i == 0 || i >= sh.n || v[j] != prev) ? i : last;
        rs[j] = last;
        prev = v[j];
    }
    const int inc = wave_incl_max(last);
    if (lane == 63)
        S.wtot[wave] = inc;
    __syncthreads();
    int pre = carry;
    for (int w = 0; w < wave; w++) {
        const int t = S.wtot[w];
        pre = pre > t ? pre : t;
    }
    {
        int excl = (int)LF_DPP_KEEP(inc, 0x138, 0xF);
        excl = lane ? excl : -1;
        pre = pre > excl ? pre : excl;
    }
#pragma unroll
    for (int j = 0; j < 4; j++)
        rs[j] = rs[j] < 0 ? pre : rs[j];
    *(int4 *)&s_rs[q0] = make_int4(rs[0], rs[1], rs[2], rs[3]);
    __syncthreads();

    const int last_q = sh.n - 1 - tb;
    uint32_t lit[4], r[4];
    bool need[4], any_need = false;
    int s4v[4], hq[4];
#pragma unroll
    for (int j = 0; j < 4; j++) {
        const int q = q0 + j;
        const bool valid = q < kEmitSpan && q <= last_q;
        const bool wraps = v[j] == 0xFFFFFFFFu;
        const bool phantom = wraps && tb + q == 0;
        const int c = (tb + q - rs[j] + (wraps && rs[j] == 0 ? 1 : 0)) & 127;
        const int s4 = q - c + 4;
        const bool same4 = c <= 3 && s4 <= last_q && s_rs[s4 < kScanSpan ? s4 : kScanSpan - 1] == rs[j];
        lit[j] = valid && (c == 0 || (c <= 3 && !same4 && !wraps));
        need[j] = valid && (c == 0 || phantom) && same4;
        r[j] = 0;
        s4v[j] = s4;
        hq[j] = q - c;
        any_need |= need[j];
    }
    if (__any(any_need)) {
#pragma unroll
        for (int j = 0; j < 4; j++) {
            const int q = q0 + j;
            int lo = need[j] ? s4v[j] : 0, hi = hq[j] + 127 < last_q ? hq[j] + 127 : last_q;
            hi = need[j] ? hi : 0;
#pragma unroll
            for (int it = 0; it < 7; it++) {
                const int mid = (lo + hi + 1) >> 1;
                const bool in_run = s_rs[mid] == rs[j];
                lo = in_run ? mid : lo;
                hi = in_run ? hi : mid - 1;
            }
            r[j] = need[j] ? (uint32_t)(lo - hq[j]) : 0u;
        }
    }
    uint32_t residue_bits = 0;
#pragma unroll
    for (int j = 0; j < 4; j++) {
        if (lit[j]) {
            uint32_t token, nb, res;
            lf_hybrid(v[j], token, nb, res);
            atomicAdd(&s_hist[token], 1u);
            residue_bits += nb;
        }
        if (r[j])
            atomicAdd(&s_hist[256u + r[j] - 3u], 1u);
    }
    if (!(HYDK_LF_PROBE & 4) && q0 < kEmitSpan && q0 <= last_q) {
        ulonglong2 *dst = (ulonglong2 *)(recs + tb + q0);
        dst[0] = make_ulonglong2(q0 + 0 <= last_q ? LF_REC(v[0], lit[0], r[0]) : 0ull, q0 + 1 <= last_q ? LF_REC(v[1], lit[1], r[1]) : 0ull);
        dst[1] = make_ulonglong2(q0 + 2 <= last_q ? LF_REC(v[2], lit[2], r[2]) : 0ull, q0 + 3 <= last_q ? LF_REC(v[3], lit[3], r[3]) : 0ull);
    }
    __syncthreads();
    return residue_bits;
}

constexpr int kPackWords = (31 + kEmitSpan * 59) / 32 + 2;

__device__ __forceinline__ uint32_t lf_window_strings(const LfShape &sh, const unsigned long long *__restrict__ recs, int tb,
                                                      const uint32_t *s_code, unsigned long long (&val)[4], uint32_t (&len)[4]) {
    const int i0 = tb + (int)threadIdx.x * 4;
    unsigned long long rec[4] = {0, 0, 0, 0};
    const bool mine_window = (int)threadIdx.x * 4 < kEmitSpan;
    if (mine_window && i0 < sh.n) {
        const ulonglong2 a = ((const ulonglong2 *)(recs + i0))[0], b = ((const ulonglong2 *)(recs + i0))[1];
        rec[0] = a.x;
        rec[1] = a.y;
        rec[2] = b.x;
        rec[3] = b.y;
    }
    uint32_t mine = 0;
#pragma unroll
    for (int j = 0; j < 4; j++) {
        val[j] = 0;
        len[j] = 0;
        if (mine_window && i0 + j < sh.n) {
            const uint32_t v = (uint32_t)rec[j], lit = (uint32_t)(rec[j] >> 32) & 1u, r = (uint32_t)(rec[j] >> 33) & 127u;
            if (lit) {
                uint32_t token, nb, res;
                lf_hybrid(v, token, nb, res);
                const uint32_t e = s_code[token];
                val[j] = (e & 0xFFFFu) | ((unsigned long long)res << (e >> 16));
                len[j] = (e >> 16) + nb;
            }
            if (r) {
                const uint32_t e = s_code[256u + r - 3u];
                val[j] |= (unsigned long long)(e & 0xFFFFu) << len[j];
                len[j] += e >> 16;
            }
        }
        mine += len[j];
    }
    return mine;
}

__global__ __launch_bounds__(kLfThreads) void k_lf_tokens(const HydkLfJob *__restrict__ jobs,
                                                          unsigned long long *__restrict__ recs_all,
                                                          uint32_t *__restrict__ hist_all, LfWork *__restrict__ work) {
    if (!(HYDK_LF_PROBE & 1))
        __builtin_amdgcn_s_setprio(3);
    const int slot = blockIdx.y, tid = threadIdx.x;
    const HydkLfJob &job = jobs[slot];
    const LfShape sh = lf_shape(job);
    __shared__ __attribute__((aligned(16))) int s_rs[kScanSpan];
    __shared__ uint32_t s_hist[HYDK_LF_CODES];
    __shared__ LfTokenScratch s_tok;
    __shared__ uint32_t s_rbits;
    if (HYDK_LF_PROBE & 8)
        return;
    for (int win = (int)blockIdx.x * HYDK_LF_WPB; win < ((int)blockIdx.x + 1) * HYDK_LF_WPB && win < kMaxWindows; win++) {
        const int tb = win * kEmitSpan;
        if (tb >= sh.n)
            return;
        if (tid == 0)
            s_rbits = 0;
        uint32_t rb = lf_tokens_window(job, sh, recs_all + (size_t)slot * HYDK_LF_SYMBOLS, tb, s_rs, s_hist, s_tok);
        rb = lf_wave_incl_sum(rb);
        if ((tid & 63) == 63 && rb)
            atomicAdd(&s_rbits, rb);
        __syncthreads();
        LfWork &w = work[slot];
        for (int i = tid; i < HYDK_LF_CODES && !(HYDK_LF_PROBE & 2); i += kLfThreads) {
            const uint32_t c = s_hist[i];
            w.win_hist[win][i] = (uint16_t)c;
            if (c)
                atomicAdd(&hist_all[(size_t)slot * HYDK_LF_CODES + i], c);
        }
        if (tid == 0)
            w.win_residue_bits[win] = s_rbits;
        if (HYDK_LF_WPB > 1)
            __syncthreads();
    }
}

__global__ __launch_bounds__(64) void k_lf_codes(const HydkLfJob *__restrict__ jobs, const uint32_t *__restrict__ hist_all,
                                                 HydkLfStream *__restrict__ streams, LfWork *__restrict__ work) {
    if (!(HYDK_LF_PROBE & 1))
        __builtin_amdgcn_s_setprio(3);
    __shared__ LfHuffScratch s_huff;
    const int slot = blockIdx.x;
    lf_code_and_offsets_wave(hist_all + (size_t)slot * HYDK_LF_CODES, work[slot], streams + slot, jobs[slot], s_huff, (int)threadIdx.x);
}

__global__ __launch_bounds__(kLfThreads) void k_lf_pack(const HydkLfJob *__restrict__ jobs,
                                                        const unsigned long long *__restrict__ recs_all,
                                                        const LfWork *__restrict__ work,
                                                        const HydkLfStream *__restrict__ streams, uint32_t *__restrict__ bits_all) {
    if (!(HYDK_LF_PROBE & 1))
        __builtin_amdgcn_s_setprio(3);
    const int slot = blockIdx.y, tid = threadIdx.x, lane = tid & 63, wave = tid >> 6;
    const LfShape sh = lf_shape(jobs[slot]);
    __shared__ uint32_t s_bits[kPackWords];
    __shared__ uint32_t s_code[HYDK_LF_CODES];
    __shared__ uint32_t s_wsum[kLfWaves];
    if ((int)blockIdx.x * HYDK_LF_WPB * kEmitSpan >= sh.n)
        return;
    for (int i = tid; i < HYDK_LF_CODES; i += kLfThreads)
        s_code[i] = work[slot].codes[i];
  for (int win = (int)blockIdx.x * HYDK_LF_WPB; win < ((int)blockIdx.x + 1) * HYDK_LF_WPB && win < kMaxWindows; win++) {
    const int tb = win * kEmitSpan;
    if (tb >= sh.n)
        return;
    if (win != (int)blockIdx.x * HYDK_LF_WPB)
        __syncthreads();
    for (int w = tid; w < kPackWords; w += kLfThreads)
        s_bits[w] = 0;
    __syncthreads();
    unsigned long long val[4];
    uint32_t len[4];
    const uint32_t mine = lf_window_strings(sh, recs_all + (size_t)slot * HYDK_LF_SYMBOLS, tb, s_code, val, len);
    const uint32_t inc = lf_wave_incl_sum(mine);
    if (lane == 63)
        s_wsum[wave] = inc;
    __syncthreads();
    const uint32_t gbits = work[slot].win_off[win];
    uint32_t pos = (gbits & 31u) + inc - mine, total = 0;
    for (int w = 0; w < kLfWaves; w++) {
        const uint32_t t = s_wsum[w];
        if (w < wave)
            pos += t;
        total += t;
    }
#pragma unroll
    for (int j = 0; j < 4; j++) {
        if (!len[j])
            continue;
        const uint32_t w = pos >> 5, shl = pos & 31u;
        const unsigned long long lo = val[j] << shl;
        const uint32_t hi = shl ? (uint32_t)(val[j] >> (64u - shl)) : 0u;
        if ((uint32_t)lo)
            atomicOr(&s_bits[w], (uint32_t)lo);
        if ((uint32_t)(lo >> 32))
            atomicOr(&s_bits[w + 1], (uint32_t)(lo >> 32));
        if (hi)
            atomicOr(&s_bits[w + 2], hi);
        pos += len[j];
    }
    __syncthreads();
    if (!total)
        continue;
    const uint32_t end = (gbits & 31u) + total, last = (end - 1u) >> 5;
    if ((gbits >> 5) + last >= (uint32_t)HYDK_LF_BITWORDS)
        continue;
    const bool ends_stream = gbits + total == streams[slot].bit_count;
    uint32_t *dst = bits_all + (size_t)slot * HYDK_LF_BITWORDS + (gbits >> 5);
    for (uint32_t w = tid; w <= last; w += kLfThreads) {
        uint32_t mask = 0xFFFFFFFFu;
        if (w == 0)
            mask <<= gbits & 31u;
        if (w == last && (end & 31u) && !ends_stream)
            mask &= (1u << (end & 31u)) - 1u;
        if (mask == 0xFFFFFFFFu)
            dst[w] = s_bits[w];
        else {
            atomicAnd(&dst[w], ~mask);
            atomicOr(&dst[w], s_bits[w]);
        }
    }
  }
}

__global__ __launch_bounds__(256) void k_lf_gather(HydkLfStream *__restrict__ streams, const uint32_t *__restrict__ bits_all,
                                                   uint32_t *__restrict__ packed, unsigned long long *__restrict__ total,
                                                   int num_slots) {
    const int slot = blockIdx.x, tid = threadIdx.x;
    __shared__ uint32_t s_off;
    if (tid < 64) {
        uint32_t mine = 0;
        for (int s = tid; s < slot; s += 64)
            mine += (streams[s].bit_count + 31u) >> 5;
#pragma unroll
        for (int d = 32; d >= 1; d >>= 1)
            mine += __shfl_xor(mine, d);
        if (tid == 0)
            s_off = mine;
    }
    __syncthreads();
    const uint32_t off = s_off, words = (streams[slot].bit_count + 31u) >> 5;
    const uint32_t *src = bits_all + (size_t)slot * HYDK_LF_BITWORDS;
    for (uint32_t w = tid; w < words; w += 256)
        packed[off + w] = src[w];
    if (tid == 0) {
        streams[slot].offset = off * 4u;
        if (slot == num_slots - 1)
            *total = (unsigned long long)(off + words) * 4ull;
    }
}

__global__ __launch_bounds__(64) void k_lf_huffman(const uint32_t *__restrict__ hist, HydkLfStream *__restrict__ stream_out,
                                                   uint32_t *__restrict__ codes) {
    __shared__ LfHuffScratch s_huff;
    uint32_t len6[kEntries];
    lf_huffman_wave(hist, codes, stream_out, s_huff, (int)threadIdx.x, len6);
}

}

namespace hydk {

size_t lf_work_bytes() { return sizeof(LfWork); }

hipError_t launch_lf_front(const HydkLfJob *d_jobs, unsigned long long *recs, uint32_t *hist, void *work, int num_slots,
                           hipStream_t stream) {
    hipLaunchKernelGGL(k_lf_tokens, dim3((kMaxWindows + HYDK_LF_WPB - 1) / HYDK_LF_WPB, num_slots), dim3(kLfThreads), 0, stream, d_jobs, recs, hist, (LfWork *)work);
    return hipGetLastError();
}

hipError_t launch_lf_codes(const HydkLfJob *d_jobs, const uint32_t *hist, HydkLfStream *streams, void *work, int num_slots,
                           hipStream_t stream) {
    hipLaunchKernelGGL(k_lf_codes, dim3(num_slots), dim3(64), 0, stream, d_jobs, hist, streams, (LfWork *)work);
    return hipGetLastError();
}

hipError_t launch_lf_back(const HydkLfJob *d_jobs, const unsigned long long *recs, HydkLfStream *streams, uint32_t *bits,
                          void *work, int num_slots, hipStream_t stream) {
    LfWork *w = (LfWork *)work;
    hipLaunchKernelGGL(k_lf_pack, dim3((kMaxWindows + HYDK_LF_WPB - 1) / HYDK_LF_WPB, num_slots), dim3(kLfThreads), 0, stream, d_jobs, recs, w,
                       streams, bits);
    return hipGetLastError();
}

hipError_t launch_lf_coder(const HydkLfJob *d_jobs, unsigned long long *recs, uint32_t *hist, HydkLfStream *streams,
                           uint32_t *bits, void *work, int num_slots, hipStream_t stream) {
    hipError_t e = launch_lf_front(d_jobs, recs, hist, work, num_slots, stream);
    if (e == hipSuccess)
        e = launch_lf_codes(d_jobs, hist, streams, work, num_slots, stream);
    if (e == hipSuccess)
        e = launch_lf_back(d_jobs, recs, streams, bits, work, num_slots, stream);
    return e;
}

hipError_t launch_lf_gather(HydkLfStream *streams, const uint32_t *bits, uint32_t *packed, unsigned long long *total,
                            int num_slots, hipStream_t stream) {
    hipLaunchKernelGGL(k_lf_gather, dim3(num_slots), dim3(256), 0, stream, streams, bits, packed, total, num_slots);
    return hipGetLastError();
}

hipError_t launch_lf_huffman_only(const uint32_t *hist, HydkLfStream *stream_out, uint32_t *codes, hipStream_t stream) {
    hipLaunchKernelGGL(k_lf_huffman, dim3(1), dim3(64), 0, stream, hist, stream_out, codes);
    return hipGetLastError();
}

}
```

Before: 101,400.

## Fold LF tokenization into tables kernel and LF packing into rANS emit

LF token generation now runs as extra workgroups of the tables kernel, and LF bit packing writes straight into the packed LF area inside the rANS emit kernel. This removes the separate LF front, back and gather launches and their serialization on the main stream. It adds a new direct-mode state flag that changes which buffer LF readback uses, plus a lazy fallback that stages the old back pass when needed. The tables kernel now shares one raw LDS buffer sized for the largest role, which may affect occupancy.

```diff
diff --git a/hydrium_amd/csrc/hip/device_api.hip b/hydrium_amd/csrc/hip/device_api.hip
--- a/hydrium_amd/csrc/hip/device_api.hip
+++ b/hydrium_amd/csrc/hip/device_api.hip
@@ -22,8 +22,9 @@
 hipError_t launch_transform(const HydkLfJob *d_jobs, int num_slots, unsigned fmt_mask, int xmode, uint32_t *status,
                             uint2 *part_info, int plog, hipStream_t stream);
 hipError_t launch_tables(const uint32_t *hist, HydkTables *tabs, const uint32_t *alpha_max, int nclusters, int first_slot,
-                         int num_slots, uint32_t alpha_floor, const uint32_t *alpha_floor_dev, const uint32_t *lf_hist,
-                         HydkLfStream *lf_streams, void *lf_work, const HydkLfJob *jobs_all, hipStream_t stream);
+                         int num_slots, uint32_t alpha_floor, const uint32_t *alpha_floor_dev, uint32_t *lf_hist,
+                         HydkLfStream *lf_streams, void *lf_work, unsigned long long *lf_recs, const HydkLfJob *jobs_all,
+                         hipStream_t stream);
 hipError_t launch_export(const HydkLfJob *d_jobs, const HydkTables *tabs, const uint32_t *group_bits, const HydkLfStream *lf_streams,
                          const uint8_t *payload, const uint64_t *hf_total, const uint8_t *lf_packed,
                          const unsigned long long *lf_total, const uint32_t *status, int num_slots, int lf_coded, uint8_t *dst,
@@ -45,7 +46,8 @@
 hipError_t launch_rans_emit(const HydkLfJob *d_jobs, const uint32_t *sym_count, const uint16_t *aux, const uint16_t *flags,
                             uint32_t aux_pitch, const uint32_t *final_state, const uint32_t *group_bits, uint64_t *offsets,
                             uint8_t *payload, int num_slots, uint32_t *status, uint64_t *total, uint64_t payload_cap,
-                            hipStream_t stream);
+                            const unsigned long long *lf_recs, const void *lf_work, HydkLfStream *lf_streams, uint32_t *lf_packed,
+                            uint32_t lf_area_words, unsigned long long *lf_total, hipStream_t stream);
 hipError_t launch_frame_begin(const HydkLfJob *host_jobs, HydkLfJob *d_jobs, int count, uint32_t *accum, size_t accum_words,
                               hipStream_t stream);
 hipError_t launch_publish(const uint64_t *total, uint64_t *h_total, const unsigned long long *lf_total,
@@ -174,6 +176,7 @@
     hipEvent_t lf_fork = nullptr, lf_join = nullptr;
     bool lf_pending = false;
     bool lf_need_gather = false;
+    bool lf_direct = false;
     bool lf_results_valid = false;
     hipEvent_t lf_ready = nullptr;
     int lf_slots = 0;
@@ -1116,6 +1119,7 @@
     ctx->want_transform = ctx->want_entropy = 0;
     ctx->host_staged = 0;
     ctx->lf_need_gather = false;
+    ctx->lf_direct = false;
     ctx->lf_results_valid = false;
     ctx->lf_slots = 0;
     HIP_TRY(ctx, hipEventRecord(ctx->frame_fence, ctx->stream));
@@ -1325,6 +1329,13 @@
     return ST_OK;
 }
 
+static int stage_direct_slots(HydAmdContext *ctx, hipStream_t where) {
+    if (ctx->lf_direct && ctx->lf_coded > 0)
+        HIP_TRY(ctx, hydk::launch_lf_back(ctx->d_jobs, ctx->lf_recs, ctx->lf_streams, ctx->lf_bits, ctx->lf_work, ctx->lf_coded, where));
+    ctx->lf_direct = false;
+    return ST_OK;
+}
+
 static int lf_range(HydAmdContext *ctx, int first, int count, bool forked) {
     if (forked) {
         const int st = ensure_lf_stream(ctx);
@@ -1336,6 +1347,11 @@
     if (forked) {
         HIP_TRY(ctx, hipEventRecord(ctx->lf_fork, ctx->stream));
         HIP_TRY(ctx, hipStreamWaitEvent(ctx->lf_stream, ctx->lf_fork, 0));
+    }
+    {
+        const int st = stage_direct_slots(ctx, where);
+        if (st != ST_OK)
+            return st;
     }
     ScopedTimer timer(ctx, HYDAMD_K_LF, where);
     HIP_TRY(ctx, hydk::launch_lf_coder(ctx->d_jobs + first, ctx->lf_recs + (size_t)first * HYDK_LF_SYMBOLS,
@@ -1344,6 +1360,7 @@
                                        ctx->lf_work + (size_t)first * hydk::lf_work_bytes(), count, where));
     ctx->lf_pending = ctx->lf_pending || forked;
     ctx->lf_need_gather = true;
+    ctx->lf_direct = false;
     return ST_OK;
 }
 
@@ -2075,17 +2092,29 @@
 static void launch_chain_standins(HydAmdContext *, int) {}
 #endif
 
-static int entropy_range(HydAmdContext *ctx, int first, int count, bool with_lf_codes) {
+static bool lf_codes_ride_tables() {
+    static const bool v = getenv("HYDAMD_LF_CODES_RIDE") && !strcmp(getenv("HYDAMD_LF_CODES_RIDE"), "tables");
+    return v;
+}
+
+static int entropy_range(HydAmdContext *ctx, int first, int count, bool with_lf_codes, bool with_lf_tokens) {
     const size_t G = HYDK_GROUPS_PER_LFG, g0 = (size_t)first * G;
+    if (with_lf_tokens && (debug_skip() & 1)) {
+        ScopedTimer timer(ctx, HYDAMD_K_LF);
+        HIP_TRY(ctx, hydk::launch_lf_front(ctx->d_jobs + first, ctx->lf_recs + (size_t)first * HYDK_LF_SYMBOLS,
+                                           ctx->lf_hist + (size_t)first * HYDK_LF_CODES,
+                                           ctx->lf_work + (size_t)first * hydk::lf_work_bytes(), count, ctx->stream));
+    }
     {
         ScopedTimer timer(ctx, HYDAMD_K_TABLES);
         if (!(debug_skip() & 1)) {
-        static const bool ride_with_tables = getenv("HYDAMD_LF_CODES_RIDE") && !strcmp(getenv("HYDAMD_LF_CODES_RIDE"), "tables");
-        const bool here = with_lf_codes && ride_with_tables;
+        const bool here = with_lf_codes && !with_lf_tokens && lf_codes_ride_tables();
         HIP_TRY(ctx, hydk::launch_tables(ctx->hist, ctx->tables, ctx->alpha_max, ctx->nclusters, first, count,
                                          ctx->alpha_floor, ctx->alpha_floor_dev,
-                                         here ? ctx->lf_hist + (size_t)first * HYDK_LF_CODES : nullptr, ctx->lf_streams + first,
-                                         ctx->lf_work + (size_t)first * hydk::lf_work_bytes(), ctx->d_jobs, ctx->stream));
+                                         here || with_lf_tokens ? ctx->lf_hist + (size_t)first * HYDK_LF_CODES : nullptr,
+                                         ctx->lf_streams + first, ctx->lf_work + (size_t)first * hydk::lf_work_bytes(),
+                                         with_lf_tokens ? ctx->lf_recs + (size_t)first * HYDK_LF_SYMBOLS : nullptr, ctx->d_jobs,
+                                         ctx->stream));
         if (here)
             with_lf_codes = false;
         }
@@ -2145,6 +2174,7 @@
     ctx->results_valid = false;
     ctx->want_entropy = num_slots;
     int lf_first = -1, lf_count = 0;
+    bool lf_tokens_ride = false;
     if (num_slots > ctx->coded && ctx->lf_on_device == 2 && ctx->rans_lanes && ctx->lf_coded == ctx->coded && !ctx->lf_pending &&
         !(debug_skip() & 8)) {
         bool any_float = false;
@@ -2153,19 +2183,24 @@
         if (!any_float) {
             lf_first = ctx->coded;
             lf_count = num_slots - ctx->coded;
-            ScopedTimer timer(ctx, HYDAMD_K_LF);
-            if (!(lf_drop() & 1))
-            HIP_TRY(ctx, hydk::launch_lf_front(ctx->d_jobs + lf_first, ctx->lf_recs + (size_t)lf_first * HYDK_LF_SYMBOLS,
-                                               ctx->lf_hist + (size_t)lf_first * HYDK_LF_CODES,
-                                               ctx->lf_work + (size_t)lf_first * hydk::lf_work_bytes(), lf_count, ctx->stream));
+            lf_tokens_ride = !lf_codes_ride_tables() && !(lf_drop() & 1);
+            if (!lf_tokens_ride && !(lf_drop() & 1)) {
+                ScopedTimer timer(ctx, HYDAMD_K_LF);
+                HIP_TRY(ctx, hydk::launch_lf_front(ctx->d_jobs + lf_first, ctx->lf_recs + (size_t)lf_first * HYDK_LF_SYMBOLS,
+                                                   ctx->lf_hist + (size_t)lf_first * HYDK_LF_CODES,
+                                                   ctx->lf_work + (size_t)lf_first * hydk::lf_work_bytes(), lf_count, ctx->stream));
+            }
         }
     }
     if (num_slots > ctx->coded) {
-        const int st = entropy_range(ctx, ctx->coded, num_slots - ctx->coded, lf_count > 0 && !(lf_drop() & 2));
+        const int st = entropy_range(ctx, ctx->coded, num_slots - ctx->coded, lf_count > 0 && !(lf_drop() & 2), lf_tokens_ride);
         if (st != ST_OK)
             return st;
         ctx->coded = num_slots;
     }
+    bool lf_direct = lf_count > 0 && lf_first == 0 && lf_count == num_slots && !(lf_drop() & (4 | 8)) && !(debug_skip() & 4);
+    for (int i = 0; i < num_slots; i++)
+        lf_direct = lf_direct && ctx->slot_lane_chain[i];
     if (!(debug_skip() & 4)) {
         ScopedTimer timer(ctx, HYDAMD_K_PACK);
         bool all_emit = true;
@@ -2174,7 +2209,9 @@
         if (all_emit)
             HIP_TRY(ctx, hydk::launch_rans_emit(ctx->d_jobs, ctx->sym_count, ctx->rans_aux, ctx->rans_flags, ctx->tok_cap,
                                                 ctx->rans_final, ctx->group_bits, ctx->offsets, ctx->payload, num_slots,
-                                                ctx->status, ctx->total, ctx->payload_cap, ctx->stream));
+                                                ctx->status, ctx->total, ctx->payload_cap, ctx->lf_recs, ctx->lf_work,
+                                                ctx->lf_streams, lf_direct ? ctx->lf_packed : nullptr,
+                                                (uint32_t)((size_t)ctx->max_slots * HYDK_LF_BITWORDS), ctx->lf_total, ctx->stream));
         else
             HIP_TRY(ctx, hydk::launch_scan(ctx->group_bits, count, ctx->offsets, ctx->total, ctx->payload, ctx->payload_cap, 1,
                                            ctx->status, ctx->stream));
@@ -2188,7 +2225,8 @@
                 HIP_TRY(ctx, hydk::launch_rans_emit(ctx->d_jobs + first, ctx->sym_count + g0, ctx->rans_aux + g0 * ctx->tok_cap,
                                                     ctx->rans_flags + g0 * (ctx->tok_cap / 16), ctx->tok_cap,
                                                     ctx->rans_final + g0, ctx->group_bits + g0, ctx->offsets + g0, ctx->payload,
-                                                    n, ctx->status, nullptr, 0, ctx->stream));
+                                                    n, ctx->status, nullptr, 0, nullptr, nullptr, nullptr, nullptr, 0, nullptr,
+                                                    ctx->stream));
             else
                 HIP_TRY(ctx, hydk::launch_pack(ctx->bitbuf + g0 * ctx->bit_pitch_words, ctx->bit_pitch_words,
                                                ctx->group_bits + g0, ctx->offsets + g0, ctx->payload,
@@ -2196,14 +2234,26 @@
             first = last + 1;
         }
     }
-    if (lf_count > 0) {
+    if (lf_direct) {
+        ctx->lf_coded = num_slots;
+        ctx->lf_slots = num_slots;
+        ctx->lf_need_gather = false;
+        ctx->lf_direct = true;
+        ctx->lf_total_unpublished = true;
+    } else if (lf_count > 0) {
         ScopedTimer timer(ctx, HYDAMD_K_LF);
+        {
+            const int st = stage_direct_slots(ctx, ctx->stream);
+            if (st != ST_OK)
+                return st;
+        }
         if (!(lf_drop() & 4))
         HIP_TRY(ctx, hydk::launch_lf_back(ctx->d_jobs + lf_first, ctx->lf_recs + (size_t)lf_first * HYDK_LF_SYMBOLS,
                                           ctx->lf_streams + lf_first, ctx->lf_bits + (size_t)lf_first * HYDK_LF_BITWORDS,
                                           ctx->lf_work + (size_t)lf_first * hydk::lf_work_bytes(), lf_count, ctx->stream));
         ctx->lf_coded = num_slots;
         ctx->lf_need_gather = true;
+        ctx->lf_direct = false;
     }
     {
         const int st = join_lf(ctx, num_slots, true);
@@ -2546,8 +2596,10 @@
     HydkLfStream h;
     HIP_TRY(ctx, hipMemcpy(&h, ctx->lf_streams + slot, sizeof(h), hipMemcpyDeviceToHost));
     const size_t have = ((size_t)h.bit_count + 7u) / 8u, n = capacity < have ? capacity : have;
+    const uint8_t *src = ctx->lf_direct ? (const uint8_t *)ctx->lf_packed + h.offset
+                                        : (const uint8_t *)(ctx->lf_bits + (size_t)slot * HYDK_LF_BITWORDS);
     if (n)
-        HIP_TRY(ctx, hipMemcpy(dst, ctx->lf_bits + (size_t)slot * HYDK_LF_BITWORDS, n, hipMemcpyDeviceToHost));
+        HIP_TRY(ctx, hipMemcpy(dst, src, n, hipMemcpyDeviceToHost));
     memset(dst + n, 0, capacity - n);
     return ST_OK;
 }
diff --git a/hydrium_amd/csrc/hip/kernels.hip b/hydrium_amd/csrc/hip/kernels.hip
--- a/hydrium_amd/csrc/hip/kernels.hip
+++ b/hydrium_amd/csrc/hip/kernels.hip
@@ -1123,6 +1123,7 @@
 }
 
 #include "lf_huffman.h"
+#include "lf_windows.h"
 
 __global__ __launch_bounds__(kThreads) void k_join_parts(const HydkLfJob *__restrict__ jobs, const uint2 *part_info, int plog,
                                                          uint32_t *status) {
@@ -1177,14 +1178,37 @@
     }
 }
 
+struct TablesLds {
+    uint32_t freq[HYDK_MAX_CLUSTERS][HYDK_ALPHABET];
+    uint32_t cutoff[HYDK_MAX_CLUSTERS][HYDK_ALPHABET];
+    uint32_t other[HYDK_MAX_CLUSTERS][HYDK_ALPHABET];
+    uint32_t shift[HYDK_MAX_CLUSTERS][HYDK_ALPHABET];
+    uint32_t base[HYDK_MAX_CLUSTERS][HYDK_ALPHABET];
+    uint8_t under[HYDK_MAX_CLUSTERS][HYDK_ALPHABET];
+    uint8_t over[HYDK_MAX_CLUSTERS][HYDK_ALPHABET];
+    uint32_t alpha[HYDK_MAX_CLUSTERS];
+    uint32_t log_alpha, err;
+};
+template <typename A, typename B, typename C>
+constexpr size_t largest_of() { return sizeof(A) > sizeof(B) ? (sizeof(A) > sizeof(C) ? sizeof(A) : sizeof(C)) : (sizeof(B) > sizeof(C) ? sizeof(B) : sizeof(C)); }
+
 __global__ __launch_bounds__(kThreads) void k_build_tables(const uint32_t *hist_all, HydkTables *tabs,
                                                            const uint32_t *alpha_max_all, int nclusters,
                                                            uint32_t alpha_floor, const uint32_t *alpha_floor_dev,
-                                                           int first_slot, int num_slots, const uint32_t *lf_hist,
-                                                           HydkLfStream *lf_streams, void *lf_work, const HydkLfJob *__restrict__ jobs_all) {
+                                                           int first_slot, int num_slots, uint32_t *lf_hist,
+                                                           HydkLfStream *lf_streams, void *lf_work, const HydkLfJob *__restrict__ jobs_all,
+                                                           unsigned long long *lf_recs) {
+    static_assert(kThreads == kLfThreads, "the LF roles are workgroups of this kernel");
+    __shared__ __attribute__((aligned(16))) unsigned char s_raw[largest_of<TablesLds, LfHuffScratch, LfTokenLds>()];
+    if ((int)blockIdx.x >= num_slots && lf_recs) {
+        const int p = (int)blockIdx.x - num_slots, s = p / kLfWorkgroups;
+        lf_tokens_role(jobs_all[first_slot + s], lf_recs + (size_t)s * HYDK_LF_SYMBOLS, lf_hist + (size_t)s * HYDK_LF_CODES,
+                       ((LfWork *)lf_work)[s], p - s * kLfWorkgroups, *(LfTokenLds *)s_raw);
+        return;
+    }
     HYDK_URGENT();
     if ((int)blockIdx.x >= num_slots) {
-        __shared__ LfHuffScratch s_huff;
+        LfHuffScratch &s_huff = *(LfHuffScratch *)s_raw;
         const int s = (int)blockIdx.x - num_slots;
         if (threadIdx.x < 64)
             lf_code_and_offsets_wave(lf_hist + (size_t)s * HYDK_LF_CODES, ((LfWork *)lf_work)[s], lf_streams + s,
@@ -1194,15 +1218,16 @@
     const unsigned slot = (unsigned)first_slot + blockIdx.x;
     const uint32_t *hist = hist_all + (size_t)slot * HYDK_MAX_CLUSTERS * HYDK_ALPHABET;
     HydkTables *tab = tabs + slot;
-    __shared__ uint32_t s_freq[HYDK_MAX_CLUSTERS][HYDK_ALPHABET];
-    __shared__ uint32_t s_cutoff[HYDK_MAX_CLUSTERS][HYDK_ALPHABET];
-    __shared__ uint32_t s_other[HYDK_MAX_CLUSTERS][HYDK_ALPHABET];
-    __shared__ uint32_t s_shift[HYDK_MAX_CLUSTERS][HYDK_ALPHABET];
-    __shared__ uint32_t s_base[HYDK_MAX_CLUSTERS][HYDK_ALPHABET];
-    __shared__ uint8_t s_under[HYDK_MAX_CLUSTERS][HYDK_ALPHABET];
-    __shared__ uint8_t s_over[HYDK_MAX_CLUSTERS][HYDK_ALPHABET];
-    __shared__ uint32_t s_alpha[HYDK_MAX_CLUSTERS];
-    __shared__ uint32_t s_log_alpha, s_err;
+    TablesLds &L = *(TablesLds *)s_raw;
+    uint32_t(&s_freq)[HYDK_MAX_CLUSTERS][HYDK_ALPHABET] = L.freq;
+    uint32_t(&s_cutoff)[HYDK_MAX_CLUSTERS][HYDK_ALPHABET] = L.cutoff;
+    uint32_t(&s_other)[HYDK_MAX_CLUSTERS][HYDK_ALPHABET] = L.other;
+    uint32_t(&s_shift)[HYDK_MAX_CLUSTERS][HYDK_ALPHABET] = L.shift;
+    uint32_t(&s_base)[HYDK_MAX_CLUSTERS][HYDK_ALPHABET] = L.base;
+    uint8_t(&s_under)[HYDK_MAX_CLUSTERS][HYDK_ALPHABET] = L.under;
+    uint8_t(&s_over)[HYDK_MAX_CLUSTERS][HYDK_ALPHABET] = L.over;
+    uint32_t(&s_alpha)[HYDK_MAX_CLUSTERS] = L.alpha;
+    uint32_t &s_log_alpha = L.log_alpha, &s_err = L.err;
 
     const int t = threadIdx.x;
     for (int i = t; i < HYDK_MAX_CLUSTERS * HYDK_ALPHABET; i += kThreads) {
@@ -2167,8 +2192,25 @@
                                                         const uint16_t *aux_all, const uint16_t *flags_all, uint32_t aux_pitch,
                                                         const uint32_t *final_state_all, const uint32_t *group_bits_all,
                                                         uint64_t *offsets_all, uint8_t *payload, uint32_t *status, int vblocks,
-                                                        uint64_t *total, uint64_t payload_cap) {
-    __shared__ uint32_t s_win[4][kEmitWin];
+                                                        uint64_t *total, uint64_t payload_cap, int lf_slots,
+                                                        const unsigned long long *__restrict__ lf_recs, const void *lf_work,
+                                                        HydkLfStream *lf_streams, uint32_t *lf_packed, uint32_t lf_area_words,
+                                                        unsigned long long *lf_total) {
+    constexpr size_t kEmitLds = sizeof(uint32_t) * 4 * kEmitWin;
+    __shared__ __attribute__((aligned(16))) unsigned char s_raw[SELF && sizeof(LfPackLds) > kEmitLds ? sizeof(LfPackLds) : kEmitLds];
+    const int emit_wgs = (int)gridDim.x - (SELF ? lf_slots * kLfWorkgroups : 0);
+    if constexpr (SELF) {
+        if ((int)blockIdx.x >= emit_wgs) {
+            LfPackLds &L = *(LfPackLds *)s_raw;
+            const int p = (int)blockIdx.x - emit_wgs, s = p / kLfWorkgroups, wg = p - s * kLfWorkgroups;
+            const uint32_t off = lf_packed_slot_offset(lf_streams, s, lf_slots, lf_total, wg, L);
+            const uint32_t left = off < lf_area_words ? lf_area_words - off : 0u;
+            lf_pack_role(jobs[s], lf_recs + (size_t)s * HYDK_LF_SYMBOLS, ((const LfWork *)lf_work)[s], lf_streams[s], lf_packed + off,
+                         left < (uint32_t)HYDK_LF_BITWORDS ? left : (uint32_t)HYDK_LF_BITWORDS, wg, L);
+            return;
+        }
+    }
+    uint32_t(&s_win)[4][kEmitWin] = *(uint32_t(*)[4][kEmitWin])s_raw;
     HYDK_URGENT();
     const int t = threadIdx.x, lane = t & 63, wave = t >> 6;
     auto wave_sum = [](uint64_t v) {
@@ -2350,7 +2392,7 @@
     if (lane == 0 && (cur & 31u))
         put(cur >> 5, carry);
     };
-    for (int vb = blockIdx.x; vb < vblocks; vb += gridDim.x)
+    for (int vb = blockIdx.x; vb < vblocks; vb += emit_wgs)
         one_block(vb);
 }
 
@@ -2631,10 +2673,14 @@
 }
 
 hipError_t launch_tables(const uint32_t *hist, HydkTables *tabs, const uint32_t *alpha_max, int nclusters, int first_slot,
-                         int num_slots, uint32_t alpha_floor, const uint32_t *alpha_floor_dev, const uint32_t *lf_hist,
-                         HydkLfStream *lf_streams, void *lf_work, const HydkLfJob *jobs_all, hipStream_t stream) {
-    hipLaunchKernelGGL(k_build_tables, dim3(lf_hist ? 2 * num_slots : num_slots), dim3(kThreads), 0, stream, hist, tabs, alpha_max,
-                       nclusters, alpha_floor, alpha_floor_dev, first_slot, num_slots, lf_hist, lf_streams, lf_work, jobs_all);
+                         int num_slots, uint32_t alpha_floor, const uint32_t *alpha_floor_dev, uint32_t *lf_hist,
+                         HydkLfStream *lf_streams, void *lf_work, unsigned long long *lf_recs, const HydkLfJob *jobs_all,
+                         hipStream_t stream) {
+    if (!lf_hist)
+        lf_recs = nullptr;
+    const int riders = !lf_hist ? 0 : lf_recs ? kLfWorkgroups * num_slots : num_slots;
+    hipLaunchKernelGGL(k_build_tables, dim3(num_slots + riders), dim3(kThreads), 0, stream, hist, tabs, alpha_max,
+                       nclusters, alpha_floor, alpha_floor_dev, first_slot, num_slots, lf_hist, lf_streams, lf_work, jobs_all, lf_recs);
     return hipGetLastError();
 }
 
@@ -2697,20 +2743,27 @@
 hipError_t launch_rans_emit(const HydkLfJob *d_jobs, const uint32_t *sym_count, const uint16_t *aux, const uint16_t *flags,
                             uint32_t aux_pitch, const uint32_t *final_state, const uint32_t *group_bits, uint64_t *offsets,
                             uint8_t *payload, int num_slots, uint32_t *status, uint64_t *total, uint64_t payload_cap,
-                            hipStream_t stream) {
+                            const unsigned long long *lf_recs, const void *lf_work, HydkLfStream *lf_streams, uint32_t *lf_packed,
+                            uint32_t lf_area_words, unsigned long long *lf_total, hipStream_t stream) {
+    if (lf_packed && !total)
+        return hipErrorInvalidValue;
     static const int share = [] {
         const char *v = getenv("HYDAMD_EMIT_SHARE");
         const int n = v && *v ? atoi(v) : HYDK_EMIT_SHARE_DEFAULT;
         return n < 1 ? 1 : n > 16 ? 16 : n;
     }();
     const int vblocks = num_slots * 16;
-    const dim3 grid((vblocks + share - 1) / share);
+    const int lf_slots = lf_packed ? num_slots : 0;
+    const dim3 grid((vblocks + share - 1) / share + lf_slots * kLfWorkgroups);
     if (total)
         hipLaunchKernelGGL(k_rans_emit<true>, grid, dim3(kThreads), 0, stream, d_jobs, sym_count, aux, flags, aux_pitch, final_state,
-                           group_bits, offsets, payload, status, vblocks, total, payload_cap);
+                           group_bits, offsets, payload, status, vblocks, total, payload_cap, lf_slots, lf_recs, lf_work, lf_streams,
+                           lf_packed, lf_area_words, lf_total);
     else
         hipLaunchKernelGGL(k_rans_emit<false>, grid, dim3(kThreads), 0, stream, d_jobs, sym_count, aux, flags, aux_pitch,
-                           final_state, group_bits, offsets, payload, status, vblocks, (uint64_t *)nullptr, (uint64_t)0);
+                           final_state, group_bits, offsets, payload, status, vblocks, (uint64_t *)nullptr, (uint64_t)0, 0,
+                           (const unsigned long long *)nullptr, (const void *)nullptr, (HydkLfStream *)nullptr, (uint32_t *)nullptr, 0u,
+                           (unsigned long long *)nullptr);
     return hipGetLastError();
 }
 
diff --git a/hydrium_amd/csrc/hip/lf_coder.hip b/hydrium_amd/csrc/hip/lf_coder.hip
--- a/hydrium_amd/csrc/hip/lf_coder.hip
+++ b/hydrium_amd/csrc/hip/lf_coder.hip
@@ -3,349 +3,19 @@
 #include <stdint.h>
 
 #include "hydk_common.h"
-#ifndef HYDK_LF_WPB
-#define HYDK_LF_WPB 1
-#endif
-#ifndef HYDK_LF_PROBE
-#define HYDK_LF_PROBE 0
-#endif
 
 namespace {
 
 #include "lf_huffman.h"
-
-constexpr int kPlane = HYDK_DC_PITCH * HYDK_DC_PITCH;
-
-#define LF_REC(v, lit, r) ((unsigned long long)(v) | ((unsigned long long)((uint32_t)(lit) | ((uint32_t)(r) << 1)) << 32))
-
-struct LfShape {
-    int vbw, blocks, n;
-    uint32_t vbw_magic;
-};
-
-__device__ __forceinline__ LfShape lf_shape(const HydkLfJob &job) {
-    LfShape sh;
-    sh.vbw = (job.width + 7) >> 3;
-    sh.blocks = sh.vbw * ((job.height + 7) >> 3);
-    sh.n = lf_values_of(job);
-    sh.vbw_magic = sh.vbw > 1 ? (uint32_t)(0xFFFFFFFFu / (uint32_t)sh.vbw) + 1u : 0u;
-    return sh;
-}
-
-__device__ __forceinline__ int lf_row_of(const LfShape &sh, int rem) {
-    return sh.vbw > 1 ? (int)__umulhi((uint32_t)rem, sh.vbw_magic) : rem;
-}
-
-__device__ __forceinline__ void lf_hybrid(uint32_t v, uint32_t &token, uint32_t &nbits, uint32_t &residue) {
-    if (v < 128u) {
-        token = v;
-        nbits = 0;
-        residue = 0;
-        return;
-    }
-    const uint32_t nb = (31u - (uint32_t)__clz(v)) - 2u;
-    residue = (v >> 1) & ((1u << nb) - 1u);
-    token = 128u + (((nb - 5u) << 2) | (((v >> (nb + 1u)) & 1u) << 1) | (v & 1u));
-    nbits = nb;
-}
-
-#define LF_DPP_KEEP(v, ctrl, rmask) ((uint32_t)__builtin_amdgcn_update_dpp((int)(v), (int)(v), ctrl, rmask, 0xF, false))
-
-__device__ __forceinline__ int wave_incl_max(int v) {
-    int t;
-    t = (int)LF_DPP_KEEP(v, 0x111, 0xF);
-    v = v > t ? v : t;
-    t = (int)LF_DPP_KEEP(v, 0x112, 0xF);
-    v = v > t ? v : t;
-    t = (int)LF_DPP_KEEP(v, 0x114, 0xF);
-    v = v > t ? v : t;
-    t = (int)LF_DPP_KEEP(v, 0x118, 0xF);
-    v = v > t ? v : t;
-    t = (int)LF_DPP_KEEP(v, 0x142, 0xA);
-    v = v > t ? v : t;
-    t = (int)LF_DPP_KEEP(v, 0x143, 0xC);
-    v = v > t ? v : t;
-    return v;
-}
-
-struct LfTokenScratch {
-    int wtot[kLfWaves];
-    uint32_t lastv[kLfWaves];
-    int head[kLfWaves];
-    uint32_t first;
-};
-
-__device__ __forceinline__ uint32_t lf_predict(int32_t cur, int32_t w, int32_t n, int32_t nw) {
-    const int32_t lo = w < n ? w : n, hi = w < n ? n : w;
-    int32_t pred = (int32_t)((uint32_t)w + (uint32_t)n - (uint32_t)nw);
-    pred = pred < lo ? lo : pred > hi ? hi : pred;
-    const uint32_t d = (uint32_t)cur - (uint32_t)pred;
-    return (d << 1) ^ (0u - (d >> 31));
-}
-
-__device__ __forceinline__ uint32_t lf_residual_at(const int32_t *dc, int c, int y, int x) {
-    const int idx = c * kPlane + y * HYDK_DC_PITCH + x;
-    const int iw = x ? idx - 1 : y ? idx - HYDK_DC_PITCH : idx;
-    const int in = y ? idx - HYDK_DC_PITCH : iw;
-    const int inw = x && y ? idx - HYDK_DC_PITCH - 1 : iw;
-    const int32_t cur = dc[idx];
-    int32_t w = dc[iw], n = dc[in], nw = dc[inw];
-    if (!(x | y))
-        w = n = nw = 0;
-    return lf_predict(cur, w, n, nw);
-}
-
-__device__ __forceinline__ uint32_t lf_value_at(const int32_t *dc, const LfShape &sh, int i) {
-    const int visit = (i >= sh.blocks) + (i >= 2 * sh.blocks);
-    const int rem = i - visit * sh.blocks;
-    const int y = lf_row_of(sh, rem), x = rem - y * sh.vbw;
-    return lf_residual_at(dc, visit < 2 ? 1 - visit : 2, y, x);
-}
-
-__device__ __forceinline__ void lf_fetch(const int32_t *dc, const LfShape &sh, int i0, uint32_t (&v)[4]) {
-#pragma unroll
-    for (int j = 0; j < 4; j++)
-        v[j] = 0;
-    if (i0 >= sh.n)
-        return;
-    int visit = (i0 >= sh.blocks) + (i0 >= 2 * sh.blocks);
-    const int rem = i0 - visit * sh.blocks;
-    int y = lf_row_of(sh, rem), x = rem - y * sh.vbw;
-    if (x + 3 < sh.vbw) {
-        const int c = visit < 2 ? 1 - visit : 2;
-        const int32_t *row = dc + c * kPlane + y * HYDK_DC_PITCH + x;
-        const int32_t *up = y ? row - HYDK_DC_PITCH : row;
-        const int32_t c0 = row[0], c1 = row[1], c2 = row[2], c3 = row[3];
-        const int32_t u0 = up[0], u1 = up[1], u2 = up[2], u3 = up[3];
-        const int32_t left = row[x ? -1 : 0], upleft = up[x ? -1 : 0];
-        const int32_t w0 = x ? left : y ? u0 : 0;
-        v[0] = lf_predict(c0, w0, y ? u0 : w0, y && x ? upleft : w0);
-        v[1] = lf_predict(c1, c0, y ? u1 : c0, y ? u0 : c0);
-        v[2] = lf_predict(c2, c1, y ? u2 : c1, y ? u1 : c1);
-        v[3] = lf_predict(c3, c2, y ? u3 : c2, y ? u2 : c2);
-        return;
-    }
-    const int vbh = sh.blocks / sh.vbw;
-#pragma unroll
-    for (int j = 0; j < 4; j++) {
-        if (visit < 3)
-            v[j] = lf_residual_at(dc, visit < 2 ? 1 - visit : 2, y, x);
-        if (++x == sh.vbw) {
-            x = 0;
-            if (++y == vbh) {
-                y = 0;
-                visit++;
-            }
-        }
-    }
-}
-
-__device__ __forceinline__ int lf_run_start(const int32_t *dc, const LfShape &sh, int from, LfTokenScratch &S) {
-    const int tid = threadIdx.x, lane = tid & 63, wave = tid >> 6;
-    for (int top = from; top >= 0; top -= kLfThreads) {
-        const int p = top - tid;
-        int head = -1;
-        if (p >= 0)
-            head = (p == 0 || lf_value_at(dc, sh, p) != lf_value_at(dc, sh, p - 1)) ? p : -1;
-        head = wave_incl_max(head);
-        if (lane == 63)
-            S.head[wave] = head;
-        __syncthreads();
-        int best = -1;
-#pragma unroll
-        for (int w = 0; w < kLfWaves; w++)
-            best = best > S.head[w] ? best : S.head[w];
-        __syncthreads();
-        if (best >= 0)
-            return best;
-    }
-    return 0;
-}
-
-__device__ __forceinline__ uint32_t lf_tokens_window(const HydkLfJob &job, const LfShape &sh, unsigned long long *__restrict__ recs,
-                                                     int tb, int *s_rs , uint32_t *s_hist, LfTokenScratch &S) {
-    const int tid = threadIdx.x, lane = tid & 63, wave = tid >> 6;
-    const int32_t *dc = job.dc;
-    const int q0 = tid * 4;
-
-    for (int i = tid; i < HYDK_LF_CODES; i += kLfThreads)
-        s_hist[i] = 0;
-    uint32_t v[4];
-    lf_fetch(dc, sh, tb + q0, v);
-    const uint32_t tailv = tb > 0 ? lf_value_at(dc, sh, tb - 1) : 0u;
-    if (lane == 63)
-        S.lastv[wave] = v[3];
-    if (tid == 0)
-        S.first = v[0];
-    __syncthreads();
-    const bool continues = tb > 0 && tb < sh.n && S.first == tailv;
-    const int carry = continues ? lf_run_start(dc, sh, tb - 1, S) : 0;
-
-    uint32_t prev = LF_DPP_KEEP(v[3], 0x138, 0xF);
-    if (lane == 0)
-        prev = wave ? S.lastv[wave - 1] : tailv;
-    int rs[4];
-    int last = -1;
-#pragma unroll
-    for (int j = 0; j < 4; j++) {
-        const int i = tb + q0 + j;
-        last = (i == 0 || i >= sh.n || v[j] != prev) ? i : last;
-        rs[j] = last;
-        prev = v[j];
-    }
-    const int inc = wave_incl_max(last);
-    if (lane == 63)
-        S.wtot[wave] = inc;
-    __syncthreads();
-    int pre = carry;
-    for (int w = 0; w < wave; w++) {
-        const int t = S.wtot[w];
-        pre = pre > t ? pre : t;
-    }
-    {
-        int excl = (int)LF_DPP_KEEP(inc, 0x138, 0xF);
-        excl = lane ? excl : -1;
-        pre = pre > excl ? pre : excl;
-    }
-#pragma unroll
-    for (int j = 0; j < 4; j++)
-        rs[j] = rs[j] < 0 ? pre : rs[j];
-    *(int4 *)&s_rs[q0] = make_int4(rs[0], rs[1], rs[2], rs[3]);
-    __syncthreads();
-
-    const int last_q = sh.n - 1 - tb;
-    uint32_t lit[4], r[4];
-    bool need[4], any_need = false;
-    int s4v[4], hq[4];
-#pragma unroll
-    for (int j = 0; j < 4; j++) {
-        const int q = q0 + j;
-        const bool valid = q < kEmitSpan && q <= last_q;
-        const bool wraps = v[j] == 0xFFFFFFFFu;
-        const bool phantom = wraps && tb + q == 0;
-        const int c = (tb + q - rs[j] + (wraps && rs[j] == 0 ? 1 : 0)) & 127;
-        const int s4 = q - c + 4;
-        const bool same4 = c <= 3 && s4 <= last_q && s_rs[s4 < kScanSpan ? s4 : kScanSpan - 1] == rs[j];
-        lit[j] = valid && (c == 0 || (c <= 3 && !same4 && !wraps));
-        need[j] = valid && (c == 0 || phantom) && same4;
-        r[j] = 0;
-        s4v[j] = s4;
-        hq[j] = q - c;
-        any_need |= need[j];
-    }
-    if (__any(any_need)) {
-#pragma unroll
-        for (int j = 0; j < 4; j++) {
-            const int q = q0 + j;
-            int lo = need[j] ? s4v[j] : 0, hi = hq[j] + 127 < last_q ? hq[j] + 127 : last_q;
-            hi = need[j] ? hi : 0;
-#pragma unroll
-            for (int it = 0; it < 7; it++) {
-                const int mid = (lo + hi + 1) >> 1;
-                const bool in_run = s_rs[mid] == rs[j];
-                lo = in_run ? mid : lo;
-                hi = in_run ? hi : mid - 1;
-            }
-            r[j] = need[j] ? (uint32_t)(lo - hq[j]) : 0u;
-        }
-    }
-    uint32_t residue_bits = 0;
-#pragma unroll
-    for (int j = 0; j < 4; j++) {
-        if (lit[j]) {
-            uint32_t token, nb, res;
-            lf_hybrid(v[j], token, nb, res);
-            atomicAdd(&s_hist[token], 1u);
-            residue_bits += nb;
-        }
-        if (r[j])
-            atomicAdd(&s_hist[256u + r[j] - 3u], 1u);
-    }
-    if (!(HYDK_LF_PROBE & 4) && q0 < kEmitSpan && q0 <= last_q) {
-        ulonglong2 *dst = (ulonglong2 *)(recs + tb + q0);
-        dst[0] = make_ulonglong2(q0 + 0 <= last_q ? LF_REC(v[0], lit[0], r[0]) : 0ull, q0 + 1 <= last_q ? LF_REC(v[1], lit[1], r[1]) : 0ull);
-        dst[1] = make_ulonglong2(q0 + 2 <= last_q ? LF_REC(v[2], lit[2], r[2]) : 0ull, q0 + 3 <= last_q ? LF_REC(v[3], lit[3], r[3]) : 0ull);
-    }
-    __syncthreads();
-    return residue_bits;
-}
-
-constexpr int kPackWords = (31 + kEmitSpan * 59) / 32 + 2;
-
-__device__ __forceinline__ uint32_t lf_window_strings(const LfShape &sh, const unsigned long long *__restrict__ recs, int tb,
-                                                      const uint32_t *s_code, unsigned long long (&val)[4], uint32_t (&len)[4]) {
-    const int i0 = tb + (int)threadIdx.x * 4;
-    unsigned long long rec[4] = {0, 0, 0, 0};
-    const bool mine_window = (int)threadIdx.x * 4 < kEmitSpan;
-    if (mine_window && i0 < sh.n) {
-        const ulonglong2 a = ((const ulonglong2 *)(recs + i0))[0], b = ((const ulonglong2 *)(recs + i0))[1];
-        rec[0] = a.x;
-        rec[1] = a.y;
-        rec[2] = b.x;
-        rec[3] = b.y;
-    }
-    uint32_t mine = 0;
-#pragma unroll
-    for (int j = 0; j < 4; j++) {
-        val[j] = 0;
-        len[j] = 0;
-        if (mine_window && i0 + j < sh.n) {
-            const uint32_t v = (uint32_t)rec[j], lit = (uint32_t)(rec[j] >> 32) & 1u, r = (uint32_t)(rec[j] >> 33) & 127u;
-            if (lit) {
-                uint32_t token, nb, res;
-                lf_hybrid(v, token, nb, res);
-                const uint32_t e = s_code[token];
-                val[j] = (e & 0xFFFFu) | ((unsigned long long)res << (e >> 16));
-                len[j] = (e >> 16) + nb;
-            }
-            if (r) {
-                const uint32_t e = s_code[256u + r - 3u];
-                val[j] |= (unsigned long long)(e & 0xFFFFu) << len[j];
-                len[j] += e >> 16;
-            }
-        }
-        mine += len[j];
-    }
-    return mine;
-}
+#include "lf_windows.h"
 
 __global__ __launch_bounds__(kLfThreads) void k_lf_tokens(const HydkLfJob *__restrict__ jobs,
                                                           unsigned long long *__restrict__ recs_all,
                                                           uint32_t *__restrict__ hist_all, LfWork *__restrict__ work) {
-    if (!(HYDK_LF_PROBE & 1))
-        __builtin_amdgcn_s_setprio(3);
-    const int slot = blockIdx.y, tid = threadIdx.x;
-    const HydkLfJob &job = jobs[slot];
-    const LfShape sh = lf_shape(job);
-    __shared__ __attribute__((aligned(16))) int s_rs[kScanSpan];
-    __shared__ uint32_t s_hist[HYDK_LF_CODES];
-    __shared__ LfTokenScratch s_tok;
-    __shared__ uint32_t s_rbits;
-    if (HYDK_LF_PROBE & 8)
-        return;
-    for (int win = (int)blockIdx.x * HYDK_LF_WPB; win < ((int)blockIdx.x + 1) * HYDK_LF_WPB && win < kMaxWindows; win++) {
-        const int tb = win * kEmitSpan;
-        if (tb >= sh.n)
-            return;
-        if (tid == 0)
-            s_rbits = 0;
-        uint32_t rb = lf_tokens_window(job, sh, recs_all + (size_t)slot * HYDK_LF_SYMBOLS, tb, s_rs, s_hist, s_tok);
-        rb = lf_wave_incl_sum(rb);
-        if ((tid & 63) == 63 && rb)
-            atomicAdd(&s_rbits, rb);
-        __syncthreads();
-        LfWork &w = work[slot];
-        for (int i = tid; i < HYDK_LF_CODES && !(HYDK_LF_PROBE & 2); i += kLfThreads) {
-            const uint32_t c = s_hist[i];
-            w.win_hist[win][i] = (uint16_t)c;
-            if (c)
-                atomicAdd(&hist_all[(size_t)slot * HYDK_LF_CODES + i], c);
-        }
-        if (tid == 0)
-            w.win_residue_bits[win] = s_rbits;
-        if (HYDK_LF_WPB > 1)
-            __syncthreads();
-    }
+    __shared__ LfTokenLds s_lds;
+    const int slot = blockIdx.y;
+    lf_tokens_role(jobs[slot], recs_all + (size_t)slot * HYDK_LF_SYMBOLS, hist_all + (size_t)slot * HYDK_LF_CODES, work[slot],
+                   (int)blockIdx.x, s_lds);
 }
 
 __global__ __launch_bounds__(64) void k_lf_codes(const HydkLfJob *__restrict__ jobs, const uint32_t *__restrict__ hist_all,
@@ -361,78 +31,10 @@
                                                         const unsigned long long *__restrict__ recs_all,
                                                         const LfWork *__restrict__ work,
                                                         const HydkLfStream *__restrict__ streams, uint32_t *__restrict__ bits_all) {
-    if (!(HYDK_LF_PROBE & 1))
-        __builtin_amdgcn_s_setprio(3);
-    const int slot = blockIdx.y, tid = threadIdx.x, lane = tid & 63, wave = tid >> 6;
-    const LfShape sh = lf_shape(jobs[slot]);
-    __shared__ uint32_t s_bits[kPackWords];
-    __shared__ uint32_t s_code[HYDK_LF_CODES];
-    __shared__ uint32_t s_wsum[kLfWaves];
-    if ((int)blockIdx.x * HYDK_LF_WPB * kEmitSpan >= sh.n)
-        return;
-    for (int i = tid; i < HYDK_LF_CODES; i += kLfThreads)
-        s_code[i] = work[slot].codes[i];
-  for (int win = (int)blockIdx.x * HYDK_LF_WPB; win < ((int)blockIdx.x + 1) * HYDK_LF_WPB && win < kMaxWindows; win++) {
-    const int tb = win * kEmitSpan;
-    if (tb >= sh.n)
-        return;
-    if (win != (int)blockIdx.x * HYDK_LF_WPB)
-        __syncthreads();
-    for (int w = tid; w < kPackWords; w += kLfThreads)
-        s_bits[w] = 0;
-    __syncthreads();
-    unsigned long long val[4];
-    uint32_t len[4];
-    const uint32_t mine = lf_window_strings(sh, recs_all + (size_t)slot * HYDK_LF_SYMBOLS, tb, s_code, val, len);
-    const uint32_t inc = lf_wave_incl_sum(mine);
-    if (lane == 63)
-        s_wsum[wave] = inc;
-    __syncthreads();
-    const uint32_t gbits = work[slot].win_off[win];
-    uint32_t pos = (gbits & 31u) + inc - mine, total = 0;
-    for (int w = 0; w < kLfWaves; w++) {
-        const uint32_t t = s_wsum[w];
-        if (w < wave)
-            pos += t;
-        total += t;
-    }
-#pragma unroll
-    for (int j = 0; j < 4; j++) {
-        if (!len[j])
-            continue;
-        const uint32_t w = pos >> 5, shl = pos & 31u;
-        const unsigned long long lo = val[j] << shl;
-        const uint32_t hi = shl ? (uint32_t)(val[j] >> (64u - shl)) : 0u;
-        if ((uint32_t)lo)
-            atomicOr(&s_bits[w], (uint32_t)lo);
-        if ((uint32_t)(lo >> 32))
-            atomicOr(&s_bits[w + 1], (uint32_t)(lo >> 32));
-        if (hi)
-            atomicOr(&s_bits[w + 2], hi);
-        pos += len[j];
-    }
-    __syncthreads();
-    if (!total)
-        continue;
-    const uint32_t end = (gbits & 31u) + total, last = (end - 1u) >> 5;
-    if ((gbits >> 5) + last >= (uint32_t)HYDK_LF_BITWORDS)
-        continue;
-    const bool ends_stream = gbits + total == streams[slot].bit_count;
-    uint32_t *dst = bits_all + (size_t)slot * HYDK_LF_BITWORDS + (gbits >> 5);
-    for (uint32_t w = tid; w <= last; w += kLfThreads) {
-        uint32_t mask = 0xFFFFFFFFu;
-        if (w == 0)
-            mask <<= gbits & 31u;
-        if (w == last && (end & 31u) && !ends_stream)
-            mask &= (1u << (end & 31u)) - 1u;
-        if (mask == 0xFFFFFFFFu)
-            dst[w] = s_bits[w];
-        else {
-            atomicAnd(&dst[w], ~mask);
-            atomicOr(&dst[w], s_bits[w]);
-        }
-    }
-  }
+    __shared__ LfPackLds s_lds;
+    const int slot = blockIdx.y;
+    lf_pack_role(jobs[slot], recs_all + (size_t)slot * HYDK_LF_SYMBOLS, work[slot], streams[slot],
+                 bits_all + (size_t)slot * HYDK_LF_BITWORDS, (uint32_t)HYDK_LF_BITWORDS, (int)blockIdx.x, s_lds);
 }
 
 __global__ __launch_bounds__(256) void k_lf_gather(HydkLfStream *__restrict__ streams, const uint32_t *__restrict__ bits_all,
@@ -477,7 +79,7 @@
 
 hipError_t launch_lf_front(const HydkLfJob *d_jobs, unsigned long long *recs, uint32_t *hist, void *work, int num_slots,
                            hipStream_t stream) {
-    hipLaunchKernelGGL(k_lf_tokens, dim3((kMaxWindows + HYDK_LF_WPB - 1) / HYDK_LF_WPB, num_slots), dim3(kLfThreads), 0, stream, d_jobs, recs, hist, (LfWork *)work);
+    hipLaunchKernelGGL(k_lf_tokens, dim3(kLfWorkgroups, num_slots), dim3(kLfThreads), 0, stream, d_jobs, recs, hist, (LfWork *)work);
     return hipGetLastError();
 }
 
@@ -490,8 +92,7 @@
 hipError_t launch_lf_back(const HydkLfJob *d_jobs, const unsigned long long *recs, HydkLfStream *streams, uint32_t *bits,
                           void *work, int num_slots, hipStream_t stream) {
     LfWork *w = (LfWork *)work;
-    hipLaunchKernelGGL(k_lf_pack, dim3((kMaxWindows + HYDK_LF_WPB - 1) / HYDK_LF_WPB, num_slots), dim3(kLfThreads), 0, stream, d_jobs, recs, w,
-                       streams, bits);
+    hipLaunchKernelGGL(k_lf_pack, dim3(kLfWorkgroups, num_slots), dim3(kLfThreads), 0, stream, d_jobs, recs, w, streams, bits);
     return hipGetLastError();
 }
 
diff --git a/hydrium_amd/csrc/hip/lf_windows.h b/hydrium_amd/csrc/hip/lf_windows.h
--- /dev/null
+++ b/hydrium_amd/csrc/hip/lf_windows.h
@@ -0,0 +1,445 @@
+#pragma once
+
+#include "lf_huffman.h"
+
+#ifndef HYDK_LF_WPB
+#define HYDK_LF_WPB 1
+#endif
+#ifndef HYDK_LF_PROBE
+#define HYDK_LF_PROBE 0
+#endif
+
+constexpr int kLfPlane = HYDK_DC_PITCH * HYDK_DC_PITCH;
+constexpr int kLfWorkgroups = (kMaxWindows + HYDK_LF_WPB - 1) / HYDK_LF_WPB;
+
+#define LF_REC(v, lit, r) ((unsigned long long)(v) | ((unsigned long long)((uint32_t)(lit) | ((uint32_t)(r) << 1)) << 32))
+
+struct LfShape {
+    int vbw, blocks, n;
+    uint32_t vbw_magic;
+};
+
+__device__ __forceinline__ LfShape lf_shape(const HydkLfJob &job) {
+    LfShape sh;
+    sh.vbw = (job.width + 7) >> 3;
+    sh.blocks = sh.vbw * ((job.height + 7) >> 3);
+    sh.n = lf_values_of(job);
+    sh.vbw_magic = sh.vbw > 1 ? (uint32_t)(0xFFFFFFFFu / (uint32_t)sh.vbw) + 1u : 0u;
+    return sh;
+}
+
+__device__ __forceinline__ int lf_row_of(const LfShape &sh, int rem) {
+    return sh.vbw > 1 ? (int)__umulhi((uint32_t)rem, sh.vbw_magic) : rem;
+}
+
+__device__ __forceinline__ void lf_hybrid(uint32_t v, uint32_t &token, uint32_t &nbits, uint32_t &residue) {
+    if (v < 128u) {
+        token = v;
+        nbits = 0;
+        residue = 0;
+        return;
+    }
+    const uint32_t nb = (31u - (uint32_t)__clz(v)) - 2u;
+    residue = (v >> 1) & ((1u << nb) - 1u);
+    token = 128u + (((nb - 5u) << 2) | (((v >> (nb + 1u)) & 1u) << 1) | (v & 1u));
+    nbits = nb;
+}
+
+#define LF_DPP_KEEP(v, ctrl, rmask) ((uint32_t)__builtin_amdgcn_update_dpp((int)(v), (int)(v), ctrl, rmask, 0xF, false))
+
+__device__ __forceinline__ int wave_incl_max(int v) {
+    int t;
+    t = (int)LF_DPP_KEEP(v, 0x111, 0xF);
+    v = v > t ? v : t;
+    t = (int)LF_DPP_KEEP(v, 0x112, 0xF);
+    v = v > t ? v : t;
+    t = (int)LF_DPP_KEEP(v, 0x114, 0xF);
+    v = v > t ? v : t;
+    t = (int)LF_DPP_KEEP(v, 0x118, 0xF);
+    v = v > t ? v : t;
+    t = (int)LF_DPP_KEEP(v, 0x142, 0xA);
+    v = v > t ? v : t;
+    t = (int)LF_DPP_KEEP(v, 0x143, 0xC);
+    v = v > t ? v : t;
+    return v;
+}
+
+struct LfTokenScratch {
+    int wtot[kLfWaves];
+    uint32_t lastv[kLfWaves];
+    int head[kLfWaves];
+    uint32_t first;
+};
+
+__device__ __forceinline__ uint32_t lf_predict(int32_t cur, int32_t w, int32_t n, int32_t nw) {
+    const int32_t lo = w < n ? w : n, hi = w < n ? n : w;
+    int32_t pred = (int32_t)((uint32_t)w + (uint32_t)n - (uint32_t)nw);
+    pred = pred < lo ? lo : pred > hi ? hi : pred;
+    const uint32_t d = (uint32_t)cur - (uint32_t)pred;
+    return (d << 1) ^ (0u - (d >> 31));
+}
+
+__device__ __forceinline__ uint32_t lf_residual_at(const int32_t *dc, int c, int y, int x) {
+    const int idx = c * kLfPlane + y * HYDK_DC_PITCH + x;
+    const int iw = x ? idx - 1 : y ? idx - HYDK_DC_PITCH : idx;
+    const int in = y ? idx - HYDK_DC_PITCH : iw;
+    const int inw = x && y ? idx - HYDK_DC_PITCH - 1 : iw;
+    const int32_t cur = dc[idx];
+    int32_t w = dc[iw], n = dc[in], nw = dc[inw];
+    if (!(x | y))
+        w = n = nw = 0;
+    return lf_predict(cur, w, n, nw);
+}
+
+__device__ __forceinline__ uint32_t lf_value_at(const int32_t *dc, const LfShape &sh, int i) {
+    const int visit = (i >= sh.blocks) + (i >= 2 * sh.blocks);
+    const int rem = i - visit * sh.blocks;
+    const int y = lf_row_of(sh, rem), x = rem - y * sh.vbw;
+    return lf_residual_at(dc, visit < 2 ? 1 - visit : 2, y, x);
+}
+
+__device__ __forceinline__ void lf_fetch(const int32_t *dc, const LfShape &sh, int i0, uint32_t (&v)[4]) {
+#pragma unroll
+    for (int j = 0; j < 4; j++)
+        v[j] = 0;
+    if (i0 >= sh.n)
+        return;
+    int visit = (i0 >= sh.blocks) + (i0 >= 2 * sh.blocks);
+    const int rem = i0 - visit * sh.blocks;
+    int y = lf_row_of(sh, rem), x = rem - y * sh.vbw;
+    if (x + 3 < sh.vbw) {
+        const int c = visit < 2 ? 1 - visit : 2;
+        const int32_t *row = dc + c * kLfPlane + y * HYDK_DC_PITCH + x;
+        const int32_t *up = y ? row - HYDK_DC_PITCH : row;
+        const int32_t c0 = row[0], c1 = row[1], c2 = row[2], c3 = row[3];
+        const int32_t u0 = up[0], u1 = up[1], u2 = up[2], u3 = up[3];
+        const int32_t left = row[x ? -1 : 0], upleft = up[x ? -1 : 0];
+        const int32_t w0 = x ? left : y ? u0 : 0;
+        v[0] = lf_predict(c0, w0, y ? u0 : w0, y && x ? upleft : w0);
+        v[1] = lf_predict(c1, c0, y ? u1 : c0, y ? u0 : c0);
+        v[2] = lf_predict(c2, c1, y ? u2 : c1, y ? u1 : c1);
+        v[3] = lf_predict(c3, c2, y ? u3 : c2, y ? u2 : c2);
+        return;
+    }
+    const int vbh = sh.blocks / sh.vbw;
+#pragma unroll
+    for (int j = 0; j < 4; j++) {
+        if (visit < 3)
+            v[j] = lf_residual_at(dc, visit < 2 ? 1 - visit : 2, y, x);
+        if (++x == sh.vbw) {
+            x = 0;
+            if (++y == vbh) {
+                y = 0;
+                visit++;
+            }
+        }
+    }
+}
+
+__device__ __forceinline__ int lf_run_start(const int32_t *dc, const LfShape &sh, int from, LfTokenScratch &S) {
+    const int tid = threadIdx.x, lane = tid & 63, wave = tid >> 6;
+    for (int top = from; top >= 0; top -= kLfThreads) {
+        const int p = top - tid;
+        int head = -1;
+        if (p >= 0)
+            head = (p == 0 || lf_value_at(dc, sh, p) != lf_value_at(dc, sh, p - 1)) ? p : -1;
+        head = wave_incl_max(head);
+        if (lane == 63)
+            S.head[wave] = head;
+        __syncthreads();
+        int best = -1;
+#pragma unroll
+        for (int w = 0; w < kLfWaves; w++)
+            best = best > S.head[w] ? best : S.head[w];
+        __syncthreads();
+        if (best >= 0)
+            return best;
+    }
+    return 0;
+}
+
+__device__ __forceinline__ uint32_t lf_tokens_window(const HydkLfJob &job, const LfShape &sh, unsigned long long *__restrict__ recs,
+                                                     int tb, int *s_rs , uint32_t *s_hist, LfTokenScratch &S) {
+    const int tid = threadIdx.x, lane = tid & 63, wave = tid >> 6;
+    const int32_t *dc = job.dc;
+    const int q0 = tid * 4;
+
+    for (int i = tid; i < HYDK_LF_CODES; i += kLfThreads)
+        s_hist[i] = 0;
+    uint32_t v[4];
+    lf_fetch(dc, sh, tb + q0, v);
+    const uint32_t tailv = tb > 0 ? lf_value_at(dc, sh, tb - 1) : 0u;
+    if (lane == 63)
+        S.lastv[wave] = v[3];
+    if (tid == 0)
+        S.first = v[0];
+    __syncthreads();
+    const bool continues = tb > 0 && tb < sh.n && S.first == tailv;
+    const int carry = continues ? lf_run_start(dc, sh, tb - 1, S) : 0;
+
+    uint32_t prev = LF_DPP_KEEP(v[3], 0x138, 0xF);
+    if (lane == 0)
+        prev = wave ? S.lastv[wave - 1] : tailv;
+    int rs[4];
+    int last = -1;
+#pragma unroll
+    for (int j = 0; j < 4; j++) {
+        const int i = tb + q0 + j;
+        last = (i == 0 || i >= sh.n || v[j] != prev) ? i : last;
+        rs[j] = last;
+        prev = v[j];
+    }
+    const int inc = wave_incl_max(last);
+    if (lane == 63)
+        S.wtot[wave] = inc;
+    __syncthreads();
+    int pre = carry;
+    for (int w = 0; w < wave; w++) {
+        const int t = S.wtot[w];
+        pre = pre > t ? pre : t;
+    }
+    {
+        int excl = (int)LF_DPP_KEEP(inc, 0x138, 0xF);
+        excl = lane ? excl : -1;
+        pre = pre > excl ? pre : excl;
+    }
+#pragma unroll
+    for (int j = 0; j < 4; j++)
+        rs[j] = rs[j] < 0 ? pre : rs[j];
+    *(int4 *)&s_rs[q0] = make_int4(rs[0], rs[1], rs[2], rs[3]);
+    __syncthreads();
+
+    const int last_q = sh.n - 1 - tb;
+    uint32_t lit[4], r[4];
+    bool need[4], any_need = false;
+    int s4v[4], hq[4];
+#pragma unroll
+    for (int j = 0; j < 4; j++) {
+        const int q = q0 + j;
+        const bool valid = q < kEmitSpan && q <= last_q;
+        const bool wraps = v[j] == 0xFFFFFFFFu;
+        const bool phantom = wraps && tb + q == 0;
+        const int c = (tb + q - rs[j] + (wraps && rs[j] == 0 ? 1 : 0)) & 127;
+        const int s4 = q - c + 4;
+        const bool same4 = c <= 3 && s4 <= last_q && s_rs[s4 < kScanSpan ? s4 : kScanSpan - 1] == rs[j];
+        lit[j] = valid && (c == 0 || (c <= 3 && !same4 && !wraps));
+        need[j] = valid && (c == 0 || phantom) && same4;
+        r[j] = 0;
+        s4v[j] = s4;
+        hq[j] = q - c;
+        any_need |= need[j];
+    }
+    if (__any(any_need)) {
+#pragma unroll
+        for (int j = 0; j < 4; j++) {
+            int lo = need[j] ? s4v[j] : 0, hi = hq[j] + 127 < last_q ? hq[j] + 127 : last_q;
+            hi = need[j] ? hi : 0;
+#pragma unroll
+            for (int it = 0; it < 7; it++) {
+                const int mid = (lo + hi + 1) >> 1;
+                const bool in_run = s_rs[mid] == rs[j];
+                lo = in_run ? mid : lo;
+                hi = in_run ? hi : mid - 1;
+            }
+            r[j] = need[j] ? (uint32_t)(lo - hq[j]) : 0u;
+        }
+    }
+    uint32_t residue_bits = 0;
+#pragma unroll
+    for (int j = 0; j < 4; j++) {
+        if (lit[j]) {
+            uint32_t token, nb, res;
+            lf_hybrid(v[j], token, nb, res);
+            atomicAdd(&s_hist[token], 1u);
+            residue_bits += nb;
+        }
+        if (r[j])
+            atomicAdd(&s_hist[256u + r[j] - 3u], 1u);
+    }
+    if (!(HYDK_LF_PROBE & 4) && q0 < kEmitSpan && q0 <= last_q) {
+        ulonglong2 *dst = (ulonglong2 *)(recs + tb + q0);
+        dst[0] = make_ulonglong2(q0 + 0 <= last_q ? LF_REC(v[0], lit[0], r[0]) : 0ull, q0 + 1 <= last_q ? LF_REC(v[1], lit[1], r[1]) : 0ull);
+        dst[1] = make_ulonglong2(q0 + 2 <= last_q ? LF_REC(v[2], lit[2], r[2]) : 0ull, q0 + 3 <= last_q ? LF_REC(v[3], lit[3], r[3]) : 0ull);
+    }
+    __syncthreads();
+    return residue_bits;
+}
+
+struct LfTokenLds {
+    __attribute__((aligned(16))) int rs[kScanSpan];
+    uint32_t hist[HYDK_LF_CODES];
+    LfTokenScratch tok;
+    uint32_t rbits;
+};
+
+__device__ __forceinline__ void lf_tokens_role(const HydkLfJob &job, unsigned long long *__restrict__ recs, uint32_t *__restrict__ hist,
+                                               LfWork &w, int wg, LfTokenLds &L) {
+    if (!(HYDK_LF_PROBE & 1))
+        __builtin_amdgcn_s_setprio(3);
+    if (HYDK_LF_PROBE & 8)
+        return;
+    const int tid = threadIdx.x;
+    const LfShape sh = lf_shape(job);
+    for (int win = wg * HYDK_LF_WPB; win < (wg + 1) * HYDK_LF_WPB && win < kMaxWindows; win++) {
+        const int tb = win * kEmitSpan;
+        if (tb >= sh.n)
+            return;
+        if (tid == 0)
+            L.rbits = 0;
+        uint32_t rb = lf_tokens_window(job, sh, recs, tb, L.rs, L.hist, L.tok);
+        rb = lf_wave_incl_sum(rb);
+        if ((tid & 63) == 63 && rb)
+            atomicAdd(&L.rbits, rb);
+        __syncthreads();
+        for (int i = tid; i < HYDK_LF_CODES && !(HYDK_LF_PROBE & 2); i += kLfThreads) {
+            const uint32_t c = L.hist[i];
+            w.win_hist[win][i] = (uint16_t)c;
+            if (c)
+                atomicAdd(&hist[i], c);
+        }
+        if (tid == 0)
+            w.win_residue_bits[win] = L.rbits;
+        if (HYDK_LF_WPB > 1)
+            __syncthreads();
+    }
+}
+
+constexpr int kPackWords = (31 + kEmitSpan * 59) / 32 + 2;
+
+__device__ __forceinline__ uint32_t lf_window_strings(const LfShape &sh, const unsigned long long *__restrict__ recs, int tb,
+                                                      const uint32_t *s_code, unsigned long long (&val)[4], uint32_t (&len)[4]) {
+    const int i0 = tb + (int)threadIdx.x * 4;
+    unsigned long long rec[4] = {0, 0, 0, 0};
+    const bool mine_window = (int)threadIdx.x * 4 < kEmitSpan;
+    if (mine_window && i0 < sh.n) {
+        const ulonglong2 a = ((const ulonglong2 *)(recs + i0))[0], b = ((const ulonglong2 *)(recs + i0))[1];
+        rec[0] = a.x;
+        rec[1] = a.y;
+        rec[2] = b.x;
+        rec[3] = b.y;
+    }
+    uint32_t mine = 0;
+#pragma unroll
+    for (int j = 0; j < 4; j++) {
+        val[j] = 0;
+        len[j] = 0;
+        if (mine_window && i0 + j < sh.n) {
+            const uint32_t v = (uint32_t)rec[j], lit = (uint32_t)(rec[j] >> 32) & 1u, r = (uint32_t)(rec[j] >> 33) & 127u;
+            if (lit) {
+                uint32_t token, nb, res;
+                lf_hybrid(v, token, nb, res);
+                const uint32_t e = s_code[token];
+                val[j] = (e & 0xFFFFu) | ((unsigned long long)res << (e >> 16));
+                len[j] = (e >> 16) + nb;
+            }
+            if (r) {
+                const uint32_t e = s_code[256u + r - 3u];
+                val[j] |= (unsigned long long)(e & 0xFFFFu) << len[j];
+                len[j] += e >> 16;
+            }
+        }
+        mine += len[j];
+    }
+    return mine;
+}
+
+struct LfPackLds {
+    uint32_t bits[kPackWords];
+    uint32_t code[HYDK_LF_CODES];
+    uint32_t wsum[kLfWaves];
+    uint32_t slot_off;
+};
+
+__device__ __forceinline__ void lf_pack_role(const HydkLfJob &job, const unsigned long long *__restrict__ recs, const LfWork &w,
+                                             const HydkLfStream &st, uint32_t *__restrict__ dst, uint32_t room, int wg, LfPackLds &L) {
+    if (!(HYDK_LF_PROBE & 1))
+        __builtin_amdgcn_s_setprio(3);
+    const int tid = threadIdx.x, lane = tid & 63, wave = tid >> 6;
+    const LfShape sh = lf_shape(job);
+    if (wg * HYDK_LF_WPB * kEmitSpan >= sh.n)
+        return;
+    for (int i = tid; i < HYDK_LF_CODES; i += kLfThreads)
+        L.code[i] = w.codes[i];
+    for (int win = wg * HYDK_LF_WPB; win < (wg + 1) * HYDK_LF_WPB && win < kMaxWindows; win++) {
+        const int tb = win * kEmitSpan;
+        if (tb >= sh.n)
+            return;
+        if (win != wg * HYDK_LF_WPB)
+            __syncthreads();
+        for (int i = tid; i < kPackWords; i += kLfThreads)
+            L.bits[i] = 0;
+        __syncthreads();
+        unsigned long long val[4];
+        uint32_t len[4];
+        const uint32_t mine = lf_window_strings(sh, recs, tb, L.code, val, len);
+        const uint32_t inc = lf_wave_incl_sum(mine);
+        if (lane == 63)
+            L.wsum[wave] = inc;
+        __syncthreads();
+        const uint32_t gbits = w.win_off[win];
+        uint32_t pos = (gbits & 31u) + inc - mine, total = 0;
+        for (int i = 0; i < kLfWaves; i++) {
+            const uint32_t t = L.wsum[i];
+            if (i < wave)
+                pos += t;
+            total += t;
+        }
+#pragma unroll
+        for (int j = 0; j < 4; j++) {
+            if (!len[j])
+                continue;
+            const uint32_t at = pos >> 5, shl = pos & 31u;
+            const unsigned long long lo = val[j] << shl;
+            const uint32_t hi = shl ? (uint32_t)(val[j] >> (64u - shl)) : 0u;
+            if ((uint32_t)lo)
+                atomicOr(&L.bits[at], (uint32_t)lo);
+            if ((uint32_t)(lo >> 32))
+                atomicOr(&L.bits[at + 1], (uint32_t)(lo >> 32));
+            if (hi)
+                atomicOr(&L.bits[at + 2], hi);
+            pos += len[j];
+        }
+        __syncthreads();
+        if (!total)
+            continue;
+        const uint32_t end = (gbits & 31u) + total, last = (end - 1u) >> 5;
+        if ((gbits >> 5) + last >= room)
+            continue;
+        const bool ends_stream = gbits + total == st.bit_count;
+        uint32_t *out = dst + (gbits >> 5);
+        for (uint32_t i = tid; i <= last; i += kLfThreads) {
+            uint32_t mask = 0xFFFFFFFFu;
+            if (i == 0)
+                mask <<= gbits & 31u;
+            if (i == last && (end & 31u) && !ends_stream)
+                mask &= (1u << (end & 31u)) - 1u;
+            if (mask == 0xFFFFFFFFu)
+                out[i] = L.bits[i];
+            else {
+                atomicAnd(&out[i], ~mask);
+                atomicOr(&out[i], L.bits[i]);
+            }
+        }
+    }
+}
+
+__device__ __forceinline__ uint32_t lf_packed_slot_offset(HydkLfStream *streams, int slot, int num_slots,
+                                                          unsigned long long *total, int wg, LfPackLds &L) {
+    const int tid = threadIdx.x;
+    if (tid < 64) {
+        uint32_t mine = 0;
+        for (int s = tid; s < slot; s += 64)
+            mine += (streams[s].bit_count + 31u) >> 5;
+        mine = lf_wave_incl_sum(mine);
+        if (tid == 63)
+            L.slot_off = mine;
+    }
+    __syncthreads();
+    const uint32_t off = L.slot_off;
+    if (wg == 0 && tid == 0) {
+        streams[slot].offset = off * 4u;
+        if (slot == num_slots - 1)
+            *total = (unsigned long long)(off + ((streams[slot].bit_count + 31u) >> 5)) * 4ull;
+    }
+    return off;
+}
```

Result: faster. 102,900, median of 6 (+1.5%).
